# invictus717/MetaTransformer

Measured on AMD Instinct MI355X. Metric: encoder samples/sec at B=256,N=197,C=768 (Base), higher is better.
Workload: dtype bf16; 1 GPU; BASELINE config 2: Meta-Transformer-Base forward+backward+AdamW, tokens [256,197,768] bf16 per GPU, 12L/768d/12h, fp32 master weights, random init N(0,0.02); mode=train, per_gpu_batch=256, global_batch=256, parallelism=single

## Files before the change

### include/metaenc.h

```cpp
#ifndef METAENC_H
#define METAENC_H

#include <stddef.h>
#include <stdint.h>

#ifdef __cplusplus
extern "C" {
#endif

#define ME_ABI_VERSION 1

enum { ME_F32 = 0, ME_BF16 = 1,
       ME_F16 = 2 ,
       ME_BF16X3 = 3 ,
       ME_BF16X2 = 4 ,
       ME_GG8 = 5  };

enum { ME_OK = 0, ME_ERR_ARG = -1, ME_ERR_UNSUPPORTED = -2, ME_ERR_HIP = -3, ME_ERR_WORKSPACE = -4 };

int me_abi_version(void);
const char* me_last_error(void);
const char* me_build_arch(void);
int me_device_info(int dev, int* num_cus, int* lds_bytes, int* clock_mhz, char* name, int name_len);

int me_row_stats(const void* x, int x_dtype, float* out, int64_t rows, int cols, float eps, void* stream);
size_t me_row_stats_partial_bytes(int64_t rows, int cols);
int me_row_stats_combine(const float* partials, int64_t rows, int cols, float eps, float* out, void* stream);
int me_layernorm_fwd(const void* x, int x_dtype, const float* gamma, const float* beta,
                     void* y, int y_dtype, float* mean, float* rstd,
                     int64_t rows, int cols, float eps, void* stream);

size_t me_layernorm_bwd_workspace(int cols);
int me_layernorm_bwd(const void* dy, int dy_dtype, const void* x, int x_dtype,
                     const float* mean, const float* rstd, const float* gamma,
                     const void* dres, int dres_dtype, void* dx, int dx_dtype,
                     float* dgamma, float* dbeta, int accumulate_affine,
                     int64_t rows, int cols, void* workspace, void* stream);

enum { ME_GEMM_NT = 0, ME_GEMM_TN = 1 };
enum { ME_ACT_NONE = 0, ME_ACT_GELU = 1 };
enum { ME_GEMM_SAVE_GELU_GRAD = 1, ME_GEMM_AUX_IS_FACTOR = 2 };

typedef struct me_gemm_desc {
    int32_t op;
    int32_t ab_dtype;
    int64_t M, N, K;
    const void* A; int64_t lda;
    const void* B; int64_t ldb;
    void* C; int64_t ldc; int32_t c_dtype;
    int32_t act;
    float alpha, beta;
    const float* bias;
    const float* colscale;
    void* preact; int64_t ldpre; int32_t preact_dtype;
    int32_t aux_dtype;
    const void* aux; int64_t ldaux;
    const void* residual; int64_t ldres; int32_t res_dtype;
    int32_t flags;
    int64_t res_row_mod;
    int64_t out_group_rows, out_group_stride, out_row_offset;
    void* workspace; int64_t workspace_bytes;
    float* colsum_a;
    const float* row_affine;
    const float* col_shift;
    float* row_stats;
    const float* row_parts;
    int32_t row_nparts;
    float row_eps;
    int64_t a_wrap_k;
} me_gemm_desc;

size_t me_gemm_workspace_bytes(const me_gemm_desc* d);
int me_gemm_fuses_colsum(const me_gemm_desc* d);
int me_gemm_emits_row_stats(const me_gemm_desc* d);
int me_gemm_reserve_cus(int cus);
int me_gemm_takes_gg8(const me_gemm_desc* d);
int me_gemm_takes_a_wrap(const me_gemm_desc* d);
int me_gemm_takes_row_parts(const me_gemm_desc* d);
int me_gemm(const me_gemm_desc* d, void* stream);

enum { ME_PROF_LN_FWD = 16, ME_PROF_LN_BWD = 17, ME_PROF_ATTN_FWD = 18, ME_PROF_ATTN_BWD = 19, ME_PROF_ROW_STATS = 20 };
typedef struct me_gemm_profile_rec {
    int32_t op, ab_dtype;
    int64_t M, N, K;
    float ms;
    int32_t plan;
} me_gemm_profile_rec;
enum { ME_ATTN_GENERIC = 1,
       ME_ATTN_TINY = 2,
       ME_ATTN_RING16 = 3,
       ME_ATTN_RESIDENT = 4,
       ME_ATTN_STREAM16 = 5,
       ME_ATTN_MID = 6,
       ME_ATTN_CHUNK = 7,
       ME_ATTN_X3 = 8,
       ME_ATTN_QKV = 9,
       ME_ATTN_DKDV32 = 16      };
int me_gemm_profile_enable(int on);
int me_gemm_profile_read(me_gemm_profile_rec* out, int max);
// ... 292 lines not shown
```

### metatransformer_amd/_capi.py

```python
from __future__ import annotations

import ctypes
import os
from ctypes import POINTER, c_char_p, c_float, c_int, c_int32, c_int64, c_size_t, c_void_p

import torch

_HERE = os.path.dirname(os.path.abspath(__file__))
LIB_PATH = os.path.join(_HERE, "libmetaenc.so")

ME_F32, ME_BF16, ME_F16 = 0, 1, 2
ME_BF16X3 = 3
ME_BF16X2 = 4
ME_GG8 = 5
ME_GEMM_NT, ME_GEMM_TN = 0, 1
ME_ACT_NONE, ME_ACT_GELU = 0, 1
ME_GEMM_SAVE_GELU_GRAD, ME_GEMM_AUX_IS_FACTOR = 1, 2
ME_PROF_LN_FWD, ME_PROF_LN_BWD, ME_PROF_ATTN_FWD, ME_PROF_ATTN_BWD, ME_PROF_ROW_STATS = 16, 17, 18, 19, 20
ME_COMM_ID_BYTES = 128
ME_RESIZE_BILINEAR, ME_RESIZE_BICUBIC = 0, 1
ME_POOL_MEAN, ME_POOL_MAX, ME_POOL_FIRST = 0, 1, 2
ME_GROUP_DP, ME_GROUP_DP_FJ, ME_GROUP_DP_DF, ME_GROUP_DP_FJ_DF = 0, 1, 2, 3
ME_GRAPH_BWD_INDEX, ME_GRAPH_BWD_GATHER = 1, 2


class MetaEncError(RuntimeError):
    pass


class GemmDesc(ctypes.Structure):
    _fields_ = [
        ("op", c_int32), ("ab_dtype", c_int32),
        ("M", c_int64), ("N", c_int64), ("K", c_int64),
        ("A", c_void_p), ("lda", c_int64),
        ("B", c_void_p), ("ldb", c_int64),
        ("C", c_void_p), ("ldc", c_int64), ("c_dtype", c_int32),
        ("act", c_int32),
        ("alpha", c_float), ("beta", c_float),
        ("bias", c_void_p),
        ("colscale", c_void_p),
        ("preact", c_void_p), ("ldpre", c_int64), ("preact_dtype", c_int32),
        ("aux_dtype", c_int32),
        ("aux", c_void_p), ("ldaux", c_int64),
        ("residual", c_void_p), ("ldres", c_int64), ("res_dtype", c_int32),
        ("flags", c_int32),
        ("res_row_mod", c_int64),
        ("out_group_rows", c_int64), ("out_group_stride", c_int64), ("out_row_offset", c_int64),
        ("workspace", c_void_p), ("workspace_bytes", c_int64),
        ("colsum_a", c_void_p),
        ("row_affine", c_void_p), ("col_shift", c_void_p),
        ("row_stats", c_void_p),
        ("row_parts", c_void_p), ("row_nparts", c_int32), ("row_eps", c_float),
        ("a_wrap_k", c_int64),
    ]


class PatchEmbedDesc(ctypes.Structure):
    _fields_ = ([("x", c_void_p), ("x_dtype", c_int32)]
                + [(n, c_int32) for n in ("B", "Cin", "T", "H", "W", "kt", "kh", "kw", "st", "sh", "sw")]
                + [("weight", c_void_p), ("w_dtype", c_int32), ("Cout", c_int32), ("bias", c_void_p),
                   ("pos", c_void_p), ("pos_dtype", c_int32), ("ld_pos", c_int64), ("prefix_rows", c_int32),
                   ("out", c_void_p), ("out_dtype", c_int32), ("ld_out", c_int64),
                   ("workspace", c_void_p), ("workspace_bytes", c_int64)])


class GraphDesc(ctypes.Structure):
    _fields_ = ([(n, c_void_p) for n in ("node_data", "edge_data", "edge_index", "offsets", "atom", "edge", "graph_token", "null_token",
                                         "order", "Z", "perturb")]
                + [(n, c_int32) for n in ("B", "T", "C", "Fn", "Fe", "Sn", "Se", "max_n", "atom_rows", "edge_rows")])


class HsiDesc(ctypes.Structure):
    _fields_ = ([("cube", c_void_p), ("cube_dtype", c_int32), ("row_stride", c_int64), ("pix_stride", c_int64)]
                + [(n, c_int32) for n in ("H", "W", "bands")] + [("points", c_void_p)]
                + [(n, c_int32) for n in ("B", "patch", "band_patch")])


class FbankDesc(ctypes.Structure):
    _fields_ = ([("wave", c_void_p), ("ld_wave", c_int64), ("lengths", c_void_p), ("wave2", c_void_p), ("ld_wave2", c_int64),
                 ("lengths2", c_void_p), ("lam", c_void_p)]
                + [(n, c_int32) for n in ("B", "n_samples", "n_samples2", "win", "shift", "padded", "n_mel", "mel_ld", "target_length")]
                + [(n, c_void_p) for n in ("window", "twiddle", "mel_range", "mel_weight", "freq_mask", "time_mask")]
                + [("normalize", c_int32), ("norm_mean", c_float), ("norm_std", c_float), ("out", c_void_p), ("out_dtype", c_int32),
                   ("ld_out", c_int64)])


class AttnQkvDesc(ctypes.Structure):
    _fields_ = ([("q", c_void_p), ("k", c_void_p), ("v", c_void_p), ("ld_q", c_int64), ("ld_k", c_int64), ("ld_v", c_int64),
                 ("out", c_void_p), ("ld_out", c_int64), ("lse", c_void_p),
                 ("dout", c_void_p), ("ld_dout", c_int64), ("delta", c_void_p),
                 ("dq", c_void_p), ("dk", c_void_p), ("dv", c_void_p), ("ld_dq", c_int64), ("ld_dk", c_int64), ("ld_dv", c_int64),
                 ("seed", ctypes.c_uint64)]
                + [(n, c_int32) for n in ("B", "Nq", "Nk", "H", "head_dim", "dtype", "causal")]
                + [("scale", c_float), ("p_drop", c_float)])


class GemmProfileRec(ctypes.Structure):
# ... 229 lines not shown
```

### metatransformer_amd/csrc/block.hip

```cpp
#include "gemm_host.h"
#include "attention_host.h"
#include <string.h>
#include <stdlib.h>
#include <atomic>
#include <map>
#include <mutex>

namespace {

struct SideCtx {
    hipStream_t side = nullptr;
    hipEvent_t fork[4] = {nullptr, nullptr, nullptr, nullptr}, join = nullptr;
    bool failed = false;
};
std::atomic<int> g_wgrad_overlap{1};
bool wgrad_overlap_on() { return g_wgrad_overlap.load() != 0; }
constexpr size_t kMaxSideCtx = 64;
SideCtx* side_ctx(hipStream_t main) {
    static std::mutex mu;
    static std::map<std::pair<int, hipStream_t>, SideCtx> ctxs;
    hipStreamCaptureStatus st = hipStreamCaptureStatusNone;
    if (hipStreamIsCapturing(main, &st) != hipSuccess || st != hipStreamCaptureStatusNone) return nullptr;
    int dev = 0;
    if (hipStreamGetDevice(main, &dev) != hipSuccess) (void)hipGetDevice(&dev);
    std::lock_guard<std::mutex> lock(mu);
    if (ctxs.size() >= kMaxSideCtx && ctxs.find(std::make_pair(dev, main)) == ctxs.end()) return nullptr;
    SideCtx& c = ctxs[std::make_pair(dev, main)];
    if (c.failed) return nullptr;
    if (!c.side) {
        int cur = dev;
        (void)hipGetDevice(&cur);
        if (cur != dev && hipSetDevice(dev) != hipSuccess) { c.failed = true; return nullptr; }
        bool ok = hipStreamCreateWithFlags(&c.side, hipStreamNonBlocking) == hipSuccess;
        for (int i = 0; ok && i < 4; ++i) ok = hipEventCreateWithFlags(&c.fork[i], hipEventDisableTiming) == hipSuccess;
        ok = ok && hipEventCreateWithFlags(&c.join, hipEventDisableTiming) == hipSuccess;
        if (cur != dev) (void)hipSetDevice(cur);
        if (!ok) { c.failed = true; c.side = nullptr; return nullptr; }
    }
    return &c;
}

inline size_t align256(size_t v) { return (v + 255) & ~(size_t)255; }

struct Dims {
    int64_t M;
    int C, C3, Hd, hd;
    size_t esz, rsz;
};
int get_dims(const me_block_desc* d, Dims& s, const char* fn) {
    ME_CHECK_ARG(d != nullptr, "%s: null descriptor", fn);
    ME_CHECK_ARG((me_dtype_ok(d->dtype) || d->dtype == ME_BF16X3) && me_dtype_ok(d->res_dtype), "%s: bad dtype", fn);
    ME_CHECK_ARG(d->B > 0 && d->N > 0 && d->C > 0 && d->heads > 0 && d->hidden > 0 && d->C % d->heads == 0,
                 "%s: bad shape B=%d N=%d C=%d heads=%d hidden=%d", fn, d->B, d->N, d->C, d->heads, d->hidden);
    s.M = (int64_t)d->B * d->N;
    s.C = d->C; s.C3 = 3 * d->C; s.Hd = d->hidden; s.hd = d->C / d->heads;
    s.esz = d->dtype == ME_BF16X3 ? 6 : me_dtype_size(d->dtype); s.rsz = me_dtype_size(d->res_dtype);
    return ME_OK;
}

struct Saved {
    char *xn1, *qkv, *o, *x1, *xn2, *hpre, *a;
    float *mean1, *rstd1, *mean2, *rstd2, *lse;
    size_t bytes;
};
Saved carve_saved(const me_block_desc* d, const Dims& s, void* base) {
    Saved v;
    size_t off = 0;
    char* b = reinterpret_cast<char*>(base);
    auto take = [&](size_t n) { char* p = b + off; off += align256(n); return p; };
    v.xn1 = take(s.M * s.C * s.esz);
    v.qkv = take(s.M * s.C3 * s.esz);
    v.o = take(s.M * s.C * s.esz);
    v.x1 = take(s.M * s.C * s.rsz);
    v.xn2 = take(s.M * s.C * s.esz);
    v.hpre = take(s.M * s.Hd * s.esz);
    v.a = take(s.M * s.Hd * s.esz);
    v.mean1 = reinterpret_cast<float*>(take(s.M * 4));
    v.rstd1 = reinterpret_cast<float*>(take(s.M * 4));
    v.mean2 = reinterpret_cast<float*>(take(s.M * 4));
    v.rstd2 = reinterpret_cast<float*>(take(s.M * 4));
    v.lse = reinterpret_cast<float*>(take((size_t)d->B * d->heads * d->N * 4));
    v.bytes = off;
    return v;
}

void gemm_desc(me_gemm_desc& g, int op, int dt, int64_t M, int64_t N, int64_t K, const void* A, int64_t lda, const void* B,
               int64_t ldb, void* C, int64_t ldc, int cdt) {
    memset(&g, 0, sizeof(g));
    g.op = op; g.ab_dtype = dt; g.M = M; g.N = N; g.K = K;
    g.A = A; g.lda = lda; g.B = B; g.ldb = ldb; g.C = C; g.ldc = ldc; g.c_dtype = cdt;
    g.alpha = 1.0f;
}

size_t gemm_scratch(const me_block_desc* d, const Dims& s, bool backward) {
    size_t w = 0;
    me_gemm_desc g;
    auto probe = [&](int op, int64_t M, int64_t N, int64_t K, int cdt, bool cs) {
        static char dummy_mem[64] __attribute__((aligned(64)));
        gemm_desc(g, op, d->dtype, M, N, K, dummy_mem, op == ME_GEMM_NT ? K : M, dummy_mem, op == ME_GEMM_NT ? K : N, dummy_mem, N, cdt);
        if (cs) g.colsum_a = reinterpret_cast<float*>(dummy_mem);
        const size_t b = me_gemm_workspace_bytes(&g);
        if (b > w) w = b;
    };
    probe(ME_GEMM_NT, s.M, s.C3, s.C, d->dtype, false);
    probe(ME_GEMM_NT, s.M, s.C, s.C, d->res_dtype, false);
    probe(ME_GEMM_NT, s.M, s.Hd, s.C, d->dtype, false);
    probe(ME_GEMM_NT, s.M, s.C, s.Hd, d->res_dtype, false);
    if (backward) {
        probe(ME_GEMM_NT, s.M, s.C, s.C3, d->dtype, false);
        probe(ME_GEMM_NT, s.M, s.C, s.Hd, d->dtype, false);
        probe(ME_GEMM_TN, s.C3, s.C, s.M, ME_F32, true);
        probe(ME_GEMM_TN, s.C, s.C, s.M, ME_F32, true);
        probe(ME_GEMM_TN, s.Hd, s.C, s.M, ME_F32, true);
        probe(ME_GEMM_TN, s.C, s.Hd, s.M, ME_F32, true);
    }
    return align256(w);
}

size_t aux_scratch(const Dims& s) {
    size_t a = me_layernorm_bwd_workspace(s.C), b = me_colsum_workspace(s.Hd > s.C3 ? s.Hd : s.C3);
    return align256(a > b ? a : b);
}

bool wants_fold(const me_block_desc* d) {
    return d->dtype != ME_BF16X3 && d->qkv_wf && d->fc1_wf && d->qkv_s && d->qkv_c && d->fc1_s && d->fc1_c && d->res_dtype == d->dtype;
}
size_t stats_scratch(const Dims& s) { return 2 * align256(me_row_stats_partial_bytes(s.M, s.C)) + 2 * align256((size_t)s.M * 8); }
bool emits_stats(const me_block_desc* d, const Dims& s) {
    if (!wants_fold(d) || d->gamma1 || d->gamma2 || s.C % ME_STATS_GROUP) return false;
    static char dummy_mem[64] __attribute__((aligned(64)));
    me_gemm_desc g;
    for (int64_t K : {(int64_t)s.C, (int64_t)s.Hd}) {
        gemm_desc(g, ME_GEMM_NT, d->dtype, s.M, s.C, K, dummy_mem, K, dummy_mem, K, dummy_mem, s.C, d->res_dtype);
        g.bias = reinterpret_cast<const float*>(dummy_mem);
        g.residual = dummy_mem; g.ldres = s.C; g.res_dtype = d->res_dtype;
        g.workspace = dummy_mem; g.workspace_bytes = (int64_t)1 << 40;
        if (!me_gemm_emits_row_stats(&g)) return false;
    }
    return true;
}

bool takes_parts(const me_block_desc* d, const Dims& s) {
    if (!wants_fold(d) || s.C % ME_STATS_GROUP || s.C > 4 * ME_STATS_GROUP) return false;
    static char dummy_mem[64] __attribute__((aligned(64)));
    me_gemm_desc g;
    for (int64_t N : {(int64_t)s.C3, (int64_t)s.Hd}) {
        gemm_desc(g, ME_GEMM_NT, d->dtype, s.M, N, s.C, dummy_mem, s.C, dummy_mem, s.C, dummy_mem, N, d->dtype);
        g.bias = reinterpret_cast<const float*>(dummy_mem);
        g.col_shift = reinterpret_cast<const float*>(dummy_mem);
        g.row_parts = reinterpret_cast<const float*>(dummy_mem); g.row_nparts = (int32_t)(s.C / ME_STATS_GROUP); g.row_eps = d->eps;
        if (N == s.Hd) g.act = ME_ACT_GELU;
        g.workspace = dummy_mem; g.workspace_bytes = (int64_t)1 << 40;
        if (!me_gemm_takes_row_parts(&g)) return false;
    }
    return true;
}

bool x3_two_planes(const Dims& s) {
// ... 217 lines not shown
    if (d->dtype == ME_BF16X3)
        return backward ? gemm_scratch_x3(s, true) + aux_scratch(s) + bwd_scratch_x3(d, s)
                        : gemm_scratch_x3(s, false) + carve_saved_x3(d, s, nullptr).bytes;
    size_t w = gemm_scratch(d, s, backward != 0) + aux_scratch(s);
    if (!backward) return w + carve_saved(d, s, nullptr).bytes + stats_scratch(s);
    w += align256(s.M * s.C * s.esz) * 4 + align256(s.M * s.Hd * s.esz) + align256(s.M * s.C * s.rsz) +
         align256(s.M * s.C3 * s.esz) + align256((size_t)d->B * d->heads * d->N * 4);
    w += align256(me_layernorm_bwd_workspace(s.C));
    return w + gemm_scratch(d, s, true) + aux_scratch(s);
}

extern "C" int me_block_fwd(const me_block_desc* d, const void* x, void* y, void* saved, void* workspace, size_t workspace_bytes,
                            void* stream) {
    Dims s;
    int rc = get_dims(d, s, "me_block_fwd");
    if (rc) return rc;
    ME_CHECK_ARG(x && y && workspace, "me_block_fwd: null pointer");
    ME_CHECK_ARG(d->qkv_w && d->proj_w && d->fc1_w && d->fc2_w && d->ln1_g && d->ln1_b && d->ln2_g && d->ln2_b,
                 "me_block_fwd: missing parameter");
    ME_CHECK_ARG(s.M * 2 * 4 <= 2 * (int64_t)align256(s.M * 4), "me_block_fwd: stash layout");
    ME_CHECK_ARG(workspace_bytes >= me_block_workspace_bytes(d, 0), "me_block_fwd: workspace too small");
    if (d->dtype == ME_BF16X3) return block_fwd_x3(d, s, x, y, saved, workspace, stream);
    char* ws = reinterpret_cast<char*>(workspace);
    const size_t gsz = gemm_scratch(d, s, false);
    void* gws = ws;
    const bool keep = saved != nullptr;
    Saved v = carve_saved(d, s, keep ? saved : ws + gsz + aux_scratch(s));
    const int dt = d->dtype, rdt = d->res_dtype;
    me_gemm_desc g;

    const bool fold = !keep && wants_fold(d);
    const bool stats = fold && emits_stats(d, s);
    const bool parts = fold && takes_parts(d, s);
    float* partials = reinterpret_cast<float*>(ws + gsz + aux_scratch(s) + v.bytes);
    if (fold) {
        gemm_desc(g, ME_GEMM_NT, dt, s.M, s.C3, s.C, x, s.C, d->qkv_wf, s.C, v.qkv, s.C3, dt);
        g.bias = d->qkv_c; g.col_shift = d->qkv_s;
        if (d->x_parts && parts) {
            g.row_parts = d->x_parts; g.row_nparts = (int32_t)(s.C / ME_STATS_GROUP); g.row_eps = d->eps;
        } else {
            const float* st1 = d->x_stats;
            if (d->x_parts) {
                if ((rc = me_row_stats_combine(d->x_parts, s.M, s.C, d->eps, v.mean1, stream))) return rc;
                st1 = v.mean1;
            } else if (!st1) {
                if ((rc = me_row_stats(x, rdt, v.mean1, s.M, s.C, d->eps, stream))) return rc;
                st1 = v.mean1;
            }
            g.row_affine = st1;
        }
    } else {
        rc = me_layernorm_fwd(x, rdt, d->ln1_g, d->ln1_b, v.xn1, dt, keep ? v.mean1 : nullptr, keep ? v.rstd1 : nullptr, s.M, s.C, d->eps, stream);
        if (rc) return rc;
        gemm_desc(g, ME_GEMM_NT, dt, s.M, s.C3, s.C, v.xn1, s.C, d->qkv_w, s.C, v.qkv, s.C3, dt);
        g.bias = d->qkv_b;
    }
    g.workspace = gws; g.workspace_bytes = (int64_t)gsz;
    if ((rc = me_gemm(&g, stream))) return rc;
    rc = me_attention_fwd(v.qkv, s.C3, v.o, s.C, keep ? v.lse : nullptr, d->B, d->N, d->heads, s.hd, d->scale, dt, 0.f, 0, stream);
    if (rc) return rc;
    gemm_desc(g, ME_GEMM_NT, dt, s.M, s.C, s.C, v.o, s.C, d->proj_w, s.C, v.x1, s.C, rdt);
    g.bias = d->proj_b; g.colscale = d->gamma1; g.residual = x; g.ldres = s.C; g.res_dtype = rdt;
    g.workspace = gws; g.workspace_bytes = (int64_t)gsz;
    if (stats) g.row_stats = partials;
    if ((rc = me_gemm(&g, stream))) return rc;
    if (fold) {
        gemm_desc(g, ME_GEMM_NT, dt, s.M, s.Hd, s.C, v.x1, s.C, d->fc1_wf, s.C, v.a, s.Hd, dt);
        g.bias = d->fc1_c; g.col_shift = d->fc1_s;
        if (stats && parts) {
            g.row_parts = partials; g.row_nparts = (int32_t)(s.C / ME_STATS_GROUP); g.row_eps = d->eps;
        } else {
            if (stats) rc = me_row_stats_combine(partials, s.M, s.C, d->eps, v.mean2, stream);
            else rc = me_row_stats(v.x1, rdt, v.mean2, s.M, s.C, d->eps, stream);
            if (rc) return rc;
            g.row_affine = v.mean2;
        }
    } else {
        rc = me_layernorm_fwd(v.x1, rdt, d->ln2_g, d->ln2_b, v.xn2, dt, keep ? v.mean2 : nullptr, keep ? v.rstd2 : nullptr, s.M, s.C, d->eps, stream);
        if (rc) return rc;
        gemm_desc(g, ME_GEMM_NT, dt, s.M, s.Hd, s.C, v.xn2, s.C, d->fc1_w, s.C, v.a, s.Hd, dt);
        g.bias = d->fc1_b;
    }
    g.act = ME_ACT_GELU;
    if (keep) { g.preact = v.hpre; g.ldpre = s.Hd; g.preact_dtype = dt; g.flags = ME_GEMM_SAVE_GELU_GRAD; }
    g.workspace = gws; g.workspace_bytes = (int64_t)gsz;
    if ((rc = me_gemm(&g, stream))) return rc;
    gemm_desc(g, ME_GEMM_NT, dt, s.M, s.C, s.Hd, v.a, s.Hd, d->fc2_w, s.Hd, y, s.C, rdt);
    g.bias = d->fc2_b; g.colscale = d->gamma2; g.residual = v.x1; g.ldres = s.C; g.res_dtype = rdt;
    g.workspace = gws; g.workspace_bytes = (int64_t)gsz;
    float* yp = d->y_parts ? d->y_parts : partials;
    if (stats && (d->y_stats || d->y_parts)) g.row_stats = yp;
    if ((rc = me_gemm(&g, stream))) return rc;
    if (stats && d->y_stats) return me_row_stats_combine(yp, s.M, s.C, d->eps, d->y_stats, stream);
    return ME_OK;
}

extern "C" int me_block_bwd(const me_block_desc* d, const void* x, const void* dy, const void* saved, void* dx,
                            const me_block_grads* gr, void* workspace, size_t workspace_bytes, void* stream) {
    Dims s;
    int rc = get_dims(d, s, "me_block_bwd");
    if (rc) return rc;
    ME_CHECK_ARG(x && dy && saved && dx && gr && workspace, "me_block_bwd: null pointer");
    ME_CHECK_ARG(dx != dy && dx != x, "me_block_bwd: dx must not alias dy or x");
    ME_CHECK_ARG(d->qkv_wt && d->proj_wt && d->fc1_wt && d->fc2_wt && d->ln1_g && d->ln2_g, "me_block_bwd: missing parameter");
    ME_CHECK_ARG(!d->gamma1 && !d->gamma2, "me_block_bwd: layer-scale backward is composed by the host (needs the unscaled branch outputs)");
    ME_CHECK_ARG(me_dtype_ok(gr->w_dtype), "me_block_bwd: bad gradient dtype");
    ME_CHECK_ARG(workspace_bytes >= me_block_workspace_bytes(d, 1), "me_block_bwd: workspace too small");
    if (d->dtype == ME_BF16X3) return block_bwd_x3(d, s, x, dy, saved, dx, gr, workspace, stream);
    const Saved v = carve_saved(d, s, const_cast<void*>(saved));
    const int dt = d->dtype, rdt = d->res_dtype;
    char* ws = reinterpret_cast<char*>(workspace);
    size_t off = 0;
    auto take = [&](size_t n) { char* p = ws + off; off += align256(n); return p; };
    const size_t gsz = gemm_scratch(d, s, true);
    void* gws = take(gsz);
    void* aws = take(aux_scratch(s));
    char* dy_c = take(s.M * s.C * s.esz);
    char* dh = take(s.M * s.Hd * s.esz);
    char* dxn = take(s.M * s.C * s.esz);
    char* dx1 = take(s.M * s.C * s.rsz);
    char* dx1_c = take(s.M * s.C * s.esz);
    char* dout = take(s.M * s.C * s.esz);
    char* dqkv = take(s.M * s.C3 * s.esz);
    float* delta = reinterpret_cast<float*>(take((size_t)d->B * d->heads * d->N * 4));
    void* ln2_ws = take(me_layernorm_bwd_workspace(s.C));
    void* gws2 = take(gsz);
    void* aws2 = take(aux_scratch(s));
    me_ln_fold_set folds[2];
    const float beta = gr->accumulate ? 1.0f : 0.0f;
    me_gemm_desc g;
    hipStream_t mstream = reinterpret_cast<hipStream_t>(stream);
    SideCtx* sc = wgrad_overlap_on() ? side_ctx(mstream) : nullptr;
    void* wstream = sc ? reinterpret_cast<void*>(sc->side) : stream;
    void* wgws = sc ? gws2 : gws;
    void* waws = sc ? aws2 : aws;
    bool forked = false;
    auto fork = [&](int i) -> int {
        if (!sc) return ME_OK;
        if (hipEventRecord(sc->fork[i], mstream) != hipSuccess || hipStreamWaitEvent(sc->side, sc->fork[i], 0) != hipSuccess) {
            me_set_error("me_block_bwd: event fork failed");
            return ME_ERR_HIP;
        }
        forked = true;
        return ME_OK;
    };
    auto join = [&](int rc_in) -> int {
        if (!sc || !forked) return rc_in;
        if (hipEventRecord(sc->join, sc->side) != hipSuccess || hipStreamWaitEvent(mstream, sc->join, 0) != hipSuccess) {
            if (rc_in == ME_OK) { me_set_error("me_block_bwd: event join failed"); return ME_ERR_HIP; }
        }
        return rc_in;
    };

    auto nt = [&](const void* A, int64_t K, const void* Wt, void* C, int64_t N, const void* aux) -> int {
        gemm_desc(g, ME_GEMM_NT, dt, s.M, N, K, A, K, Wt, K, C, N, dt);
        if (aux) { g.aux = aux; g.ldaux = N; g.aux_dtype = dt; g.flags = ME_GEMM_AUX_IS_FACTOR; }
        g.workspace = gws; g.workspace_bytes = (int64_t)gsz;
        return me_gemm(&g, stream);
    };
    auto wgrad = [&](int fk, const void* dOut, int64_t n_out, const void* In, int64_t n_in, void* dW, float* dB) -> int {
        if (!dW && !dB) return ME_OK;
        int r = fork(fk);
        if (r) return r;
        if (dW) {
            gemm_desc(g, ME_GEMM_TN, dt, n_out, n_in, s.M, dOut, n_out, In, n_in, dW, n_in, gr->w_dtype);
            g.beta = beta; g.workspace = wgws; g.workspace_bytes = (int64_t)gsz;
            const bool fuse = dB && me_gemm_fuses_colsum(&g);
            if (fuse) g.colsum_a = dB;
            r = me_gemm(&g, wstream);
            if (r) return r;
            if (fuse) return ME_OK;
        }
        if (dB) return me_colsum(dOut, dt, n_out, s.M, n_out, dB, gr->accumulate, waws, wstream);
        return ME_OK;
    };

    const void* dyc = dy;
    if (rdt != dt) {
        if ((rc = me_cast(dy, rdt, dy_c, dt, s.M * s.C, stream))) return rc;
        dyc = dy_c;
    }
    if ((rc = wgrad(0, dyc, s.C, v.a, s.Hd, gr->fc2_w, gr->fc2_b))) return join(rc);
    if ((rc = nt(dyc, s.C, d->fc2_wt, dh, s.Hd, v.hpre))) return join(rc);
    if ((rc = wgrad(1, dh, s.Hd, v.xn2, s.C, gr->fc1_w, gr->fc1_b))) return join(rc);
    if ((rc = nt(dh, s.Hd, d->fc1_wt, dxn, s.C, nullptr))) return join(rc);
    rc = me_ln_bwd_deferred(dxn, dt, v.x1, rdt, v.mean2, v.rstd2, d->ln2_g, dy, rdt, dx1, rdt, gr->ln2_g, gr->ln2_b, gr->accumulate, s.M,
                            s.C, ln2_ws, stream, &folds[0]);
    if (rc) return join(rc);
    const void* dx1c = dx1;
    if (rdt != dt) {
        if ((rc = me_cast(dx1, rdt, dx1_c, dt, s.M * s.C, stream))) return join(rc);
        dx1c = dx1_c;
    }
    if ((rc = wgrad(2, dx1c, s.C, v.o, s.C, gr->proj_w, gr->proj_b))) return join(rc);
    if ((rc = nt(dx1c, s.C, d->proj_wt, dout, s.C, nullptr))) return join(rc);
    rc = me_attention_bwd(v.qkv, s.C3, v.o, s.C, dout, s.C, v.lse, delta, dqkv, s.C3, d->B, d->N, d->heads, s.hd, d->scale, dt, 0.f, 0, stream);
    if (rc) return join(rc);
    if ((rc = wgrad(3, dqkv, s.C3, v.xn1, s.C, gr->qkv_w, gr->qkv_b))) return join(rc);
    if ((rc = nt(dqkv, s.C3, d->qkv_wt, dxn, s.C, nullptr))) return join(rc);
    rc = me_ln_bwd_deferred(dxn, dt, x, rdt, v.mean1, v.rstd1, d->ln1_g, dx1, rdt, dx, rdt, gr->ln1_g, gr->ln1_b, gr->accumulate, s.M, s.C,
                            aws, stream, &folds[1]);
    if (rc) return join(rc);
    return join(me_ln_bwd_fold_sets(folds, 2, s.C, stream));
}

extern "C" int me_block_bwd_overlap(int enable) {
    const int prev = wgrad_overlap_on() ? 1 : 0;
    g_wgrad_overlap.store(enable ? 1 : 0);
    return prev;
}

extern "C" int me_encoder_fwd(const me_block_desc* blocks, int n_blocks, const void* x, void* y, void* pingpong, void* workspace,
                              size_t workspace_bytes, void* stream) {
    ME_CHECK_ARG(blocks && n_blocks > 0 && x && y && workspace, "me_encoder_fwd: bad args");
    ME_CHECK_ARG(n_blocks == 1 || pingpong, "me_encoder_fwd: more than one block needs the ping-pong token buffer");
    const void* in = x;
    const float* st_in = nullptr;
    const float* parts_in = nullptr;
    for (int i = 0; i < n_blocks; ++i) {
        void* out = ((n_blocks - 1 - i) % 2 == 0) ? y : pingpong;
        me_block_desc d = blocks[i];
        Dims s;
        int rc = get_dims(&d, s, "me_encoder_fwd");
        if (rc) return rc;
        d.x_stats = st_in;
        d.y_stats = nullptr;
        d.x_parts = parts_in;
        d.y_parts = nullptr;
        const me_block_desc& nx = blocks[i + 1 < n_blocks ? i + 1 : i];
        const bool chain = i + 1 < n_blocks && emits_stats(&d, s) && wants_fold(&nx) && nx.C == d.C && nx.B == d.B && nx.N == d.N &&
                           nx.eps == d.eps && nx.hidden == d.hidden && nx.heads == d.heads && nx.dtype == d.dtype &&
                           nx.res_dtype == d.res_dtype && me_block_workspace_bytes(&nx, 0) == me_block_workspace_bytes(&d, 0) &&
                           workspace_bytes >= me_block_workspace_bytes(&d, 0);
        if (chain) {
            char* tail = reinterpret_cast<char*>(workspace) + me_block_workspace_bytes(&d, 0) - 2 * align256((size_t)s.M * 8);
            Dims sn;
            if (get_dims(&nx, sn, "me_encoder_fwd") == ME_OK && takes_parts(&nx, sn))
                d.y_parts = reinterpret_cast<float*>(tail - align256(me_row_stats_partial_bytes(s.M, s.C)));
            else
// ... 11 lines not shown
```

### metatransformer_amd/csrc/common.h

```cpp
#pragma once
constexpr int ME_POL_LN_ST = 0;
constexpr int ME_POL_LN_LD = 0;
constexpr int ME_POL_ATTN_ST = 0;
constexpr int ME_POL_SLAB = 0;
#define ME_NT_LOAD(POL, ptr) ((POL) ? __builtin_nontemporal_load(ptr) : *(ptr))
#define ME_NT_STORE(POL, val, ptr) do { if (POL) __builtin_nontemporal_store((val), (ptr)); else *(ptr) = (val); } while (0)
#include <hip/hip_runtime.h>
#include <stdint.h>
#include <stdio.h>
#include "../../include/metaenc.h"

typedef __bf16 bf16_t;
typedef __attribute__((ext_vector_type(8))) __bf16 bf16x8;
typedef __attribute__((ext_vector_type(4))) __bf16 bf16x4;
typedef __attribute__((ext_vector_type(2))) __bf16 bf16x2;
typedef __attribute__((ext_vector_type(16))) float f32x16;
typedef __attribute__((ext_vector_type(4))) float f32x4;
typedef __attribute__((ext_vector_type(2))) float f32x2;
typedef __attribute__((ext_vector_type(4))) uint32_t u32x4;
constexpr float ME_GG8_LO = -0.13f, ME_GG8_STEP = 1.26f / 255.0f;
constexpr int ME_STATS_GROUP = 256;
typedef __attribute__((ext_vector_type(2))) uint32_t u32x2;

#define ME_WAVE 64

void me_set_error(const char* fmt, ...);
#define ME_CHECK_ARG(cond, ...)                 \
    do {                                        \
        if (!(cond)) {                          \
            me_set_error(__VA_ARGS__);          \
            return ME_ERR_ARG;                  \
        }                                       \
    } while (0)
#define ME_CHECK_LAUNCH(name)                                                        \
    do {                                                                             \
        hipError_t e__ = hipGetLastError();                                          \
        if (e__ != hipSuccess) {                                                     \
            me_set_error("%s: launch failed: %s", name, hipGetErrorString(e__));     \
            return ME_ERR_HIP;                                                       \
        }                                                                            \
    } while (0)

struct OncePerDevice {
    bool done[64] = {};
    bool need() {
        int d = 0;
        if (hipGetDevice(&d) != hipSuccess || d < 0 || d >= 64) return true;
        if (done[d]) return false;
        done[d] = true;
        return true;
    }
};
template <auto Kernel, typename... Args>
int launch_kernel(const char* label, dim3 grid, int threads, size_t lds, size_t lds_max, hipStream_t stream, Args... args) {
    static OncePerDevice once;
    if (once.need()) (void)hipFuncSetAttribute(reinterpret_cast<const void*>(Kernel), hipFuncAttributeMaxDynamicSharedMemorySize, (int)lds_max);
    hipLaunchKernelGGL(Kernel, grid, dim3(threads), lds, stream, args...);
    ME_CHECK_LAUNCH(label);
    return ME_OK;
}

static inline int device_cus() {
    static int n = 0;
    if (!n) {
        int dev = 0;
        (void)hipGetDevice(&dev);
        if (hipDeviceGetAttribute(&n, hipDeviceAttributeMultiprocessorCount, dev) != hipSuccess || n <= 0) n = 256;
    }
    return n;
}

struct ProfScope {
    hipEvent_t e0 = nullptr;
    hipStream_t stream;
    int op, dt;
    int64_t M, N, K;
    int plan = 0;
    ProfScope(int op, int dt, int64_t M, int64_t N, int64_t K, hipStream_t stream);
    ~ProfScope();
};

static inline size_t me_dtype_size(int dt) { return dt == ME_F32 ? 4 : dt == ME_GG8 ? 1 : 2; }
static inline bool me_dtype_ok(int dt) { return dt == ME_F32 || dt == ME_BF16; }
static inline bool me_storage_dtype_ok(int dt) { return me_dtype_ok(dt) || dt == ME_F16; }
static inline bool me_out_dtype_ok(int dt) { return me_dtype_ok(dt) || dt == ME_BF16X3; }
static inline bool me_is_planes(int dt) { return dt == ME_BF16X3 || dt == ME_BF16X2; }
static inline bool aligned4(const void* p, int dt) { return (uintptr_t)p % (4 * me_dtype_size(dt)) == 0; }
constexpr int EW_THREADS = 256;
static inline unsigned grid_blocks(int64_t work_items) {
    int64_t b = (work_items + EW_THREADS - 1) / EW_THREADS;
    const int64_t cap = 256 * 8;
    return (unsigned)(b < 1 ? 1 : (b > cap ? cap : b));
}

constexpr int LN_FOLD_SETS = 4;
struct me_ln_fold_set { const float* partial; int nrows; float* dgamma; float* dbeta; int accumulate; };
struct me_ln_fold_batch { me_ln_fold_set set[LN_FOLD_SETS]; int cols; };
int me_ln_bwd_deferred(const void* dy, int dy_dtype, const void* x, int x_dtype, const float* mean, const float* rstd, const float* gamma,
                       const void* dres, int dres_dtype, void* dx, int dx_dtype, float* dgamma, float* dbeta, int accumulate_affine,
                       int64_t rows, int cols, void* workspace, void* stream, me_ln_fold_set* defer);
int me_ln_bwd_fold_sets(const me_ln_fold_set* sets, int n, int cols, void* stream);

__device__ __forceinline__ float bf16_bits_to_f32(uint32_t lo16) { return __uint_as_float(lo16 << 16); }

__device__ __forceinline__ float wave_sum(float v) {
#pragma unroll
    for (int o = 32; o > 0; o >>= 1) v += __shfl_xor(v, o, 64);
    return v;
}
__device__ __forceinline__ float wave_max(float v) {
#pragma unroll
    for (int o = 32; o > 0; o >>= 1) v = fmaxf(v, __shfl_xor(v, o, 64));
    return v;
}

__device__ __forceinline__ f32x4 load4_as_f32(const void* base, int dt, int64_t idx) {
    if (dt == ME_BF16) {
        u32x2 raw = *reinterpret_cast<const u32x2*>(reinterpret_cast<const uint16_t*>(base) + idx);
        f32x4 r;
        r[0] = __uint_as_float(raw[0] << 16);
        r[1] = __uint_as_float(raw[0] & 0xffff0000u);
        r[2] = __uint_as_float(raw[1] << 16);
        r[3] = __uint_as_float(raw[1] & 0xffff0000u);
        return r;
    }
    return *reinterpret_cast<const f32x4*>(reinterpret_cast<const float*>(base) + idx);
}
__device__ __forceinline__ void store4_from_f32(void* base, int dt, int64_t idx, f32x4 v) {
    if (dt == ME_BF16) {
        bf16x4 o;
        o[0] = (bf16_t)v[0]; o[1] = (bf16_t)v[1]; o[2] = (bf16_t)v[2]; o[3] = (bf16_t)v[3];
        *reinterpret_cast<bf16x4*>(reinterpret_cast<uint16_t*>(base) + idx) = o;
    } else {
        *reinterpret_cast<f32x4*>(reinterpret_cast<float*>(base) + idx) = v;
    }
}
__device__ __forceinline__ void store4_split3(uint16_t* row, int64_t cols, int64_t c, f32x4 v, bool right_operand = false) {
    bf16x4 h, l;
#pragma unroll
    for (int e = 0; e < 4; ++e) {
        h[e] = (bf16_t)v[e];
        l[e] = (bf16_t)(v[e] - (float)h[e]);
    }
    *reinterpret_cast<bf16x4*>(row + c) = h;
    *reinterpret_cast<bf16x4*>(row + cols + c) = right_operand ? h : l;
    *reinterpret_cast<bf16x4*>(row + 2 * cols + c) = right_operand ? l : h;
}
__device__ __forceinline__ void store4_split2(uint16_t* row, int64_t cols, int64_t c, f32x4 v) {
    bf16x4 h, l;
#pragma unroll
    for (int e = 0; e < 4; ++e) {
        h[e] = (bf16_t)v[e];
        l[e] = (bf16_t)(v[e] - (float)h[e]);
    }
    *reinterpret_cast<bf16x4*>(row + c) = h;
    *reinterpret_cast<bf16x4*>(row + cols + c) = l;
}

__device__ __forceinline__ float load1_as_f32(const void* base, int dt, int64_t idx) {
    if (dt == ME_BF16) return bf16_bits_to_f32(reinterpret_cast<const uint16_t*>(base)[idx]);
    return reinterpret_cast<const float*>(base)[idx];
}
__device__ __forceinline__ void store1_from_f32(void* base, int dt, int64_t idx, float v) {
    if (dt == ME_BF16) reinterpret_cast<bf16_t*>(base)[idx] = (bf16_t)v;
    else reinterpret_cast<float*>(base)[idx] = v;
// ... 113 lines not shown
```

### metatransformer_amd/csrc/gemm.hip

```cpp
#include "gemm_common.h"
#include <string.h>
#include <algorithm>
#include <atomic>

namespace {

constexpr int BM = 128;
constexpr int BN = 128;
constexpr int ROWB = 128;
constexpr int TILE_BYTES = BM * ROWB;
constexpr int NT = 256;

__device__ __forceinline__ int lds_off(int row, int byteoff) {
    const int chunk = byteoff >> 4;
    return row * ROWB + (((chunk ^ ((row >> 1) & 7)) << 4) | (byteoff & 15));
}

struct Stage { u32x4 v[4]; };

template <typename T>
__device__ __forceinline__ void load_nt(Stage& s, const T* __restrict__ S, int64_t ld, int64_t nrows, int64_t K,
                                        int64_t r0, int64_t k0, int tid) {
    constexpr int E = 16 / sizeof(T);
#pragma unroll
// ... 434 lines not shown
        pl.ksteps_per_split = nk;
        if (fam == GEMM_G3) {
            const int64_t tn_ = (d->N + 255) / 256, tiles4 = tm * tn_;
            const int SL = 256;
            const int64_t R4 = tiles4 / SL, rem4 = tiles4 - R4 * SL;
            const int nkt = (int)(d->K / 64);
            const bool resident = d->c_dtype == ME_BF16 && d->alpha == 1.0f;
            if (!resident && d->N <= 1024 && d->K >= 2048 && R4 >= 1 && rem4 * 20 >= SL && rem4 * 10 <= SL * 6 && d->res_row_mod == 0 &&
                d->out_group_rows == 0) {
                const int64_t m_main = (R4 * SL) / tn_;
                const int64_t tail_tiles = (tm - m_main) * tn_;
                int s = (int)(SL / tail_tiles);
                int ktp = (nkt + s - 1) / s;
                ktp += ktp & 1;
                if (s >= 2 && m_main >= 1 && ktp >= 2) {
                    pl.tail_rows = d->M - m_main * 256;
                    pl.tail_ksteps = ktp;
                    pl.tail_split = (nkt + ktp - 1) / ktp;
                    if (pl.tail_split >= 2) pl.ws_bytes = (size_t)pl.tail_split * (size_t)pl.tail_rows * (size_t)d->N * sizeof(float);
                    else pl.tail_rows = 0;
                }
            }
            return pl;
        }
        const int64_t tn_ = (d->N + pl.bn - 1) / pl.bn, tiles = tm * tn_;
        const int64_t R = tiles / SLOTS, rem = tiles - R * SLOTS;
        if (fam == GEMM_G2W && d->N <= 1024 && R >= 1 && rem * 20 >= SLOTS && rem * 10 <= SLOTS * 6 &&
            d->res_row_mod == 0 && d->out_group_rows == 0 && d->M % pl.bm == 0) {
            const int64_t m_main = (R * SLOTS) / tn_;
            const int64_t tail_tiles = (tm - m_main) * tn_;
            int s = (int)(SLOTS / tail_tiles);
            while (s > 1 && nk / s < 8) --s;
            if (s >= 2 && m_main >= 1) {
                pl.tail_rows = (tm - m_main) * pl.bm;
                pl.tail_ksteps = (nk + s - 1) / s;
                pl.tail_split = (nk + pl.tail_ksteps - 1) / pl.tail_ksteps;
                pl.ws_bytes = (size_t)pl.tail_split * (size_t)pl.tail_rows * (size_t)d->N * sizeof(float);
            }
        }
        if (pl.tail_rows == 0 && tiles * kSmallSplitDen <= SLOTS && nk >= (small_nt ? 64 : 16) &&
            (!small_nt || tiles <= 96 || nk >= kSmallSplitLongK)) {
            int s = (int)(SLOTS / tiles);
            while (s > 1 && nk / s < 8) --s;
            if (s >= 2) {
                pl.tail_rows = d->M;
                pl.tail_ksteps = (nk + s - 1) / s;
                pl.tail_split = (nk + pl.tail_ksteps - 1) / pl.tail_ksteps;
                pl.ws_bytes = (size_t)pl.tail_split * (size_t)d->M * (size_t)d->N * sizeof(float);
            }
        }
    }
    return pl;
}

int fill_params(const me_gemm_desc* d, GemmParams& p) {
    ME_CHECK_ARG(d != nullptr, "me_gemm: null descriptor");
    ME_CHECK_ARG(d->op == ME_GEMM_NT || d->op == ME_GEMM_TN, "me_gemm: bad op %d", d->op);
    ME_CHECK_ARG(me_dtype_ok(d->ab_dtype) && (me_out_dtype_ok(d->c_dtype) || d->c_dtype == ME_BF16X2), "me_gemm: bad dtype");
    if (me_is_planes(d->c_dtype))
        ME_CHECK_ARG(d->op == ME_GEMM_NT && d->beta == 0.0f && d->ldc >= (d->c_dtype == ME_BF16X3 ? 3 : 2) * d->N && d->out_group_rows == 0 && !d->colsum_a,
                     "me_gemm: ME_BF16X3 / ME_BF16X2 output: NT, beta = 0, ldc >= 3 N / 2 N, plain rows");
    ME_CHECK_ARG(d->a_wrap_k == 0 || (d->op == ME_GEMM_NT && d->ab_dtype == ME_BF16 && d->a_wrap_k > 0 && d->a_wrap_k % 128 == 0 && d->a_wrap_k < d->K &&
                                      d->K - d->a_wrap_k <= d->a_wrap_k && d->lda >= d->a_wrap_k),
                 "me_gemm: a_wrap_k: NT, bf16, a multiple of 128 with K / 2 <= a_wrap_k < K, lda >= a_wrap_k");
    ME_CHECK_ARG(d->M > 0 && d->N > 0 && d->K > 0, "me_gemm: empty problem M=%lld N=%lld K=%lld",
                 (long long)d->M, (long long)d->N, (long long)d->K);
    ME_CHECK_ARG(d->A && d->B && d->C, "me_gemm: null operand");
    const int E = d->ab_dtype == ME_BF16 ? 8 : 4;
    ME_CHECK_ARG(d->N % 4 == 0, "me_gemm: N=%lld must be a multiple of 4", (long long)d->N);
    ME_CHECK_ARG(d->ldc % 4 == 0, "me_gemm: ldc must be a multiple of 4");
    if (d->op == ME_GEMM_NT) {
        ME_CHECK_ARG(d->K % E == 0 && d->lda % E == 0 && d->ldb % E == 0,
                     "me_gemm(NT): K, lda, ldb must be multiples of %d elements (16 bytes)", E);
    } else {
        ME_CHECK_ARG(d->M % E == 0 && d->N % E == 0 && d->lda % E == 0 && d->ldb % E == 0,
                     "me_gemm(TN): M, N, lda, ldb must be multiples of %d elements (16 bytes)", E);
    }
    ME_CHECK_ARG(((uintptr_t)d->A | (uintptr_t)d->B | (uintptr_t)d->C) % 16 == 0, "me_gemm: operands must be 16-byte aligned");
    ME_CHECK_ARG(d->act == ME_ACT_NONE || d->act == ME_ACT_GELU, "me_gemm: bad act");
    ME_CHECK_ARG((d->flags & ~(ME_GEMM_SAVE_GELU_GRAD | ME_GEMM_AUX_IS_FACTOR)) == 0, "me_gemm: unknown flags");
    ME_CHECK_ARG(!(d->flags & ME_GEMM_SAVE_GELU_GRAD) || (d->act == ME_ACT_GELU && d->preact), "me_gemm: ME_GEMM_SAVE_GELU_GRAD needs act = GELU and preact");
    ME_CHECK_ARG(!(d->flags & ME_GEMM_AUX_IS_FACTOR) || d->aux, "me_gemm: ME_GEMM_AUX_IS_FACTOR needs aux");
    if (d->preact) ME_CHECK_ARG((me_dtype_ok(d->preact_dtype) && d->ldpre % 4 == 0) ||
                                (d->preact_dtype == ME_GG8 && d->flags == ME_GEMM_SAVE_GELU_GRAD && d->ldpre % 8 == 0 && (uintptr_t)d->preact % 8 == 0), "me_gemm: bad preact");
    if (d->aux) ME_CHECK_ARG((me_dtype_ok(d->aux_dtype) && d->ldaux % 4 == 0) ||
                             (d->aux_dtype == ME_GG8 && d->flags == ME_GEMM_AUX_IS_FACTOR && d->ldaux % 8 == 0 && (uintptr_t)d->aux % 8 == 0), "me_gemm: bad aux");
    if (d->residual) ME_CHECK_ARG(me_dtype_ok(d->res_dtype) && d->ldres % 4 == 0, "me_gemm: bad residual");
    p.A = d->A; p.B = d->B; p.C = d->C;
    p.M = d->M; p.N = d->N; p.K = d->K; p.lda = d->lda; p.ldb = d->ldb; p.ldc = d->ldc;
    p.c_dtype = d->c_dtype; p.act = d->act; p.alpha = d->alpha; p.beta = d->beta;
    p.bias = d->bias; p.colscale = d->colscale;
    p.preact = d->preact; p.ldpre = d->ldpre; p.preact_dtype = d->preact_dtype;
    p.flags = d->flags;
    p.aux = d->aux; p.ldaux = d->ldaux; p.aux_dtype = d->aux_dtype;
    p.residual = d->residual; p.ldres = d->ldres; p.res_dtype = d->res_dtype;
    p.res_row_mod = d->res_row_mod; p.out_group_rows = d->out_group_rows;
    p.out_group_stride = d->out_group_stride; p.out_row_offset = d->out_row_offset;
    p.split_k = 1; p.ksteps_per_split = 0;
    p.colsum_ws = nullptr;
    ME_CHECK_ARG((d->row_affine == nullptr && d->row_parts == nullptr) == (d->col_shift == nullptr), "me_gemm: row_affine (or row_parts) and col_shift go together");
    ME_CHECK_ARG(!d->row_affine || d->op == ME_GEMM_NT, "me_gemm: row_affine (folded LayerNorm) is defined for ME_GEMM_NT");
    p.row_affine = d->row_affine; p.col_shift = d->col_shift;
    p.row_nparts = 0; p.row_eps = 0.0f;
    p.sk_wgs = 0; p.sk_upt = 0; p.sk_levels = 0; p.sk_l1 = 0;
    p.a_wrap_kt = (int)(d->a_wrap_k / 64);
    if (d->row_parts) {
        ME_CHECK_ARG(!d->row_affine && d->col_shift && d->op == ME_GEMM_NT, "me_gemm: row_parts replaces row_affine (NT, with col_shift)");
        ME_CHECK_ARG(d->row_nparts >= 1 && d->row_nparts <= 4 && (int64_t)d->row_nparts * ME_STATS_GROUP == d->K && d->row_eps >= 0.0f,
                     "me_gemm: row_parts: row_nparts = K / 256, 1 .. 4 (see me_gemm_takes_row_parts)");
        ME_CHECK_ARG((uintptr_t)d->row_parts % 8 == 0, "me_gemm: row_parts must be 8-byte aligned");
        p.row_affine = d->row_parts; p.row_nparts = d->row_nparts; p.row_eps = d->row_eps;
    }
    ME_CHECK_ARG(!d->row_stats || (d->op == ME_GEMM_NT && d->residual && (uintptr_t)d->row_stats % 8 == 0),
                 "me_gemm: row_stats goes with ME_GEMM_NT and a residual operand (8-byte aligned)");
    p.row_stats = d->row_stats;
    p.g3_full_tiles = 0; p.g3_split = 0; p.g3_ktp = 0; p.g3_slabs = nullptr; p.slab_stride = 0; p.g3_tickets = nullptr; p.g3_half = 0;
    if (d->colsum_a) ME_CHECK_ARG(d->op == ME_GEMM_TN, "me_gemm: colsum_a is defined for ME_GEMM_TN only");
    p.tiles_m = (int)((d->M + BM - 1) / BM);
    p.tiles_n = (int)((d->N + BN - 1) / BN);
    ME_CHECK_ARG((int64_t)p.tiles_m * p.tiles_n < (1ll << 31), "me_gemm: too many tiles");
    return ME_OK;
}

struct GemmRoute {
    GemmParams p;
    GemmPlan pl;
    G3Form form;
    bool colsum_a = false;
    bool a_wrap = false;
    bool gg8 = false;
    bool row_parts = false;
    bool row_stats_kernel = false, row_stats = false;
};

int route_gemm(const me_gemm_desc* d, GemmRoute& r, bool allow_sk = true) {
    GemmParams& p = r.p;
    const int rc = fill_params(d, p);
    if (rc) return rc;
    const GemmPlan& pl = r.pl = plan_gemm(d, p, allow_sk);
    if (pl.family != GEMM_G128) {
        p.tiles_m = (int)((d->M + pl.bm - 1) / pl.bm);
        p.tiles_n = (int)((d->N + pl.bn - 1) / pl.bn);
    }
    r.colsum_a = d->op == ME_GEMM_TN && ((pl.family == GEMM_G2B && pl.split_k > 1) || pl.family == GEMM_G3);
    if (pl.family != GEMM_G3 || d->op != ME_GEMM_NT) return ME_OK;
    const int cus = g3_cu_count();
    r.form = g3_form(p, cus);
    r.a_wrap = r.form.kernel == G3_ONE_TILE_WRAP;
    r.gg8 = pl.tail_rows == 0 && r.form.kernel == G3_RESIDENT && r.form.pre == G3_PRE_GG8;
    GemmParams pu = p;
    pu.a_wrap_kt = 0;
    const G3Form fu = g3_form(pu, cus);
    const bool resident = pl.tail_rows == 0 && fu.kernel == G3_RESIDENT;
    r.row_parts = resident && fu.pre == G3_PRE_ROW_PARTS && p.M * 8 * 16 < (1ll << 31);
    r.row_stats_kernel = resident && fu.repi == 2;
    r.row_stats = r.row_stats_kernel && p.res_dtype == ME_BF16 && p.N % 256 == 0 && p.M * 8 < (1ll << 31);
    return ME_OK;
}

GemmParams tail_rows_of(const GemmParams& p, int64_t m1) {
    GemmParams pt = p;
    pt.M = p.M - m1;
    pt.C = reinterpret_cast<char*>(p.C) + (size_t)m1 * p.ldc * me_dtype_size(p.c_dtype);
    if (p.preact) pt.preact = reinterpret_cast<char*>(p.preact) + (size_t)m1 * p.ldpre * me_dtype_size(p.preact_dtype);
    if (p.aux) pt.aux = reinterpret_cast<const char*>(p.aux) + (size_t)m1 * p.ldaux * me_dtype_size(p.aux_dtype);
    if (p.residual) pt.residual = reinterpret_cast<const char*>(p.residual) + (size_t)m1 * p.ldres * me_dtype_size(p.res_dtype);
    if (p.row_affine) pt.row_affine = p.row_affine + 2 * m1;
    return pt;
}

int gemm_impl(const me_gemm_desc* d, hipStream_t stream, int* plan_out, GemmTnLaunch tn_launch = nullptr, const void* tn_ctx = nullptr) {
    GemmRoute r;
    int rc = route_gemm(d, r, tn_launch == nullptr);
    if (rc) return rc;
    GemmParams& p = r.p;
    const GemmPlan& pl = r.pl;
    if (tn_launch && !(pl.family == GEMM_G3 && d->op == ME_GEMM_TN)) return ME_ERR_UNSUPPORTED;
    const bool have_ws = pl.ws_bytes && d->workspace && (size_t)d->workspace_bytes >= pl.ws_bytes;
    float* const ws = reinterpret_cast<float*>(d->workspace);
    {
        const int parts = pl.split_k > 1 ? pl.split_k : (pl.tail_rows > 0 ? pl.tail_split : 1);
        *plan_out = (pl.family & 15) | ((have_ws && parts > 1) ? 16 : 0) | (pl.sk_wgs ? 32 : 0) | ((have_ws ? parts : 1) << 8);
    }
    if (d->colsum_a)
        ME_CHECK_ARG(r.colsum_a && have_ws, "me_gemm: colsum_a needs the split-K wgrad kernel and its workspace (see me_gemm_fuses_colsum)");
    if (d->row_stats)
        ME_CHECK_ARG(d->a_wrap_k ? pl.family == GEMM_G3 && d->op == ME_GEMM_NT && pl.tail_rows == 0 : r.row_stats_kernel,
                     "me_gemm: row_stats is not available for this problem (see me_gemm_emits_row_stats)");
    if (d->a_wrap_k)
        ME_CHECK_ARG(r.a_wrap, "me_gemm: a_wrap_k is not available for this problem (see me_gemm_takes_a_wrap)");
    if (d->row_parts)
        ME_CHECK_ARG(r.row_parts, "me_gemm: row_parts is not available for this problem (see me_gemm_takes_row_parts)");
    if ((d->preact && d->preact_dtype == ME_GG8) || (d->aux && d->aux_dtype == ME_GG8))
        ME_CHECK_ARG(r.gg8, "me_gemm: ME_GG8 is not available for this problem (see me_gemm_takes_gg8)");

    if (pl.family == GEMM_G3 && d->op == ME_GEMM_TN) {
        ME_CHECK_ARG(have_ws, "me_gemm(TN, g3): workspace of me_gemm_workspace_bytes() required");
        GemmParams ps = p;
        ps.C = ws;
        ps.split_k = pl.split_k;
        ps.ksteps_per_split = pl.ksteps_per_split;
        ps.slab_stride = g3_tn_slab_stride(d->M, d->N);
        if (d->colsum_a) ps.colsum_ws = ws + (size_t)pl.split_k * (size_t)ps.slab_stride;
        if (pl.sk_wgs) {
            ps.sk_wgs = pl.sk_wgs; ps.sk_upt = pl.sk_upt; ps.sk_levels = pl.sk_levels; ps.sk_l1 = pl.sk_l1;
            rc = launch_g3_tn_sk(ps, stream);
            p.sk_wgs = pl.sk_wgs; p.sk_upt = pl.sk_upt; p.sk_levels = pl.sk_levels; p.sk_l1 = pl.sk_l1;
        } else {
            rc = tn_launch ? tn_launch(ps, stream, tn_ctx) : launch_g3_tn(ps, stream);
        }
        if (rc) return rc;
        launch_splitk_reduce(p, stream, ws, pl.split_k, ps.colsum_ws, pl.split_k * p.tiles_n, d->colsum_a, ps.slab_stride);
        ME_CHECK_LAUNCH("me_gemm(g3 tn fold)");
        return ME_OK;
    }
    if (pl.family == GEMM_G3) {
        if (!(pl.tail_rows > 0 && have_ws)) return launch_g3(p, r.form, stream);
        const int64_t m1 = d->M - pl.tail_rows;
        p.g3_full_tiles = (int)(m1 / 256) * p.tiles_n;
        p.g3_split = pl.tail_split;
        p.g3_ktp = pl.tail_ksteps;
        p.g3_slabs = ws;
        rc = launch_g3(p, g3_form(p, g3_cu_count()), stream);
        if (rc) return rc;
        GemmParams pt = tail_rows_of(p, m1);
        pt.A = nullptr;
        launch_splitk_reduce(pt, stream, ws, pl.tail_split, nullptr, 0, nullptr);
        ME_CHECK_LAUNCH("me_gemm(g3 tail fold)");
        return ME_OK;
    }
    if (pl.family == GEMM_G128) {
        if (d->ab_dtype == ME_BF16)
            return d->op == ME_GEMM_NT ? launch_g128<bf16_t, false>(p, stream) : launch_g128<bf16_t, true>(p, stream);
        return d->op == ME_GEMM_NT ? launch_g128<float, false>(p, stream) : launch_g128<float, true>(p, stream);
    }
    auto run = [&](const GemmParams& q) { return launch_g2b(q, d->op, pl.bm, pl.bn, stream); };
    p.ksteps_per_split = pl.ksteps_per_split;
    if (pl.split_k > 1 && have_ws) {
        GemmParams ps = p;
        ps.C = ws;
        ps.split_k = pl.split_k;
        if (d->colsum_a) ps.colsum_ws = ws + (size_t)pl.split_k * (size_t)d->M * (size_t)d->N;
        rc = run(ps);
        if (rc) return rc;
        launch_splitk_reduce(p, stream, ws, pl.split_k, ps.colsum_ws, pl.split_k * p.tiles_n, d->colsum_a);
        ME_CHECK_LAUNCH("me_gemm(splitk reduce)");
        return ME_OK;
    }
    p.ksteps_per_split = (int)(d->K / pl.kstep);
    if (!(pl.tail_rows > 0 && have_ws)) return run(p);
    const int64_t m1 = d->M - pl.tail_rows;
    if (m1 > 0) {
        GemmParams pm = p;
        pm.M = m1;
        pm.tiles_m = (int)(m1 / pl.bm);
        rc = run(pm);
        if (rc) return rc;
    }
    GemmParams pt = tail_rows_of(p, m1);
    pt.tiles_m = (int)((pl.tail_rows + pl.bm - 1) / pl.bm);
    pt.A = reinterpret_cast<const char*>(p.A) + (size_t)m1 * p.lda * me_dtype_size(d->ab_dtype);
    GemmParams ps = pt;
    ps.C = ws;
    ps.split_k = pl.tail_split;
    ps.ksteps_per_split = pl.tail_ksteps;
    rc = run(ps);
    if (rc) return rc;
    launch_splitk_reduce(pt, stream, ws, pl.tail_split, nullptr, 0, nullptr);
    ME_CHECK_LAUNCH("me_gemm(tail fold)");
    return ME_OK;
}

}

int gemm_fill_params(const me_gemm_desc* d, GemmParams& p) { return fill_params(d, p); }

extern "C" int me_gemm(const me_gemm_desc* d, void* stream_) {
// ... 53 lines not shown
```

### metatransformer_amd/csrc/gemm3.hip

```cpp
#include "gemm3_core.h"

namespace {
constexpr int G3_ROWOP_AHEAD = 4;
constexpr int G3_ROWOP_AHEAD_HALF = 4;
constexpr int G3_ROWOP_AHEAD_STATS = 4;

template <int EPI, bool WRAP = false>
__global__ __launch_bounds__(512) __attribute__((amdgpu_waves_per_eu(2, 2))) void gemm_g3_kernel(const GemmParams p) {
    extern __shared__ __attribute__((aligned(16))) char smem[];
    const int tid = threadIdx.x, lane = tid & 63;
    const int wave = __builtin_amdgcn_readfirstlane(tid >> 6);
    const int wr = wave >> 2;

    const int nwg = gridDim.x, bid = blockIdx.x;
    const int xcd = bid & 7, slot = bid >> 3;
    const int F = p.g3_full_tiles;
    const int nf = (F >> 3) + (xcd < (F & 7) ? 1 : 0);
    const int base_f = xcd * (F >> 3) + (xcd < (F & 7) ? xcd : (F & 7));
    int tile, part = -1;
    if (slot < nf) {
        tile = base_f + slot;
    } else {
        const int base_all = xcd * (nwg >> 3) + (xcd < (nwg & 7) ? xcd : (nwg & 7));
        const int tid_ = base_all - base_f + (slot - nf);
// ... 64 lines not shown
    (void)lane;
    lane = g3_lane_now();
    const int col = tn * G3_BN + (wave & 3) * 64 + 4 * (lane >> 4);
#pragma unroll
    for (int nt = 0; nt < 4; ++nt)
        b.v[nt] = __builtin_bit_cast(f32x4, __builtin_amdgcn_raw_buffer_load_b128(brs, (col + nt * 16) * 4, 0, 0));
    return b;
}
__device__ __forceinline__ void g3r_set_binit(G3State& s, const G3Bias& b, bool zero) {
    const f32x4 z = {0.f, 0.f, 0.f, 0.f};
#pragma unroll
    for (int j = 0; j < 4; ++j) s.binit[j] = zero ? z : b.v[j];
    asm volatile("" ::"v"(s.binit[0]), "v"(s.binit[1]), "v"(s.binit[2]), "v"(s.binit[3]));
}

__device__ __forceinline__ void g3r_rows8(f32x4& x0, f32x4& x1, f32x4& y0, f32x4& y1) {
#pragma unroll
    for (int e = 0; e < 4; ++e) {
        const unsigned a0 = __float_as_uint(x0[e]), a1 = __float_as_uint(x1[e]), b0 = __float_as_uint(y0[e]), b1 = __float_as_uint(y1[e]);
        x0[e] = __uint_as_float(__builtin_amdgcn_update_dpp(a0, b0, 0x128, 0xf, 0xc, false));
        x1[e] = __uint_as_float(__builtin_amdgcn_update_dpp(a1, b1, 0x128, 0xf, 0xc, false));
        y0[e] = __uint_as_float(__builtin_amdgcn_update_dpp(b0, a0, 0x128, 0xf, 0x3, false));
        y1[e] = __uint_as_float(__builtin_amdgcn_update_dpp(b1, a1, 0x128, 0xf, 0x3, false));
    }
}

__device__ __forceinline__ void g3r_rows8_packed(u32x4& x, u32x4& y) {
#pragma unroll
    for (int e = 0; e < 4; ++e) {
        const unsigned a = x[e], b = y[e];
        x[e] = __builtin_amdgcn_update_dpp(a, b, 0x128, 0xf, 0xc, false);
        y[e] = __builtin_amdgcn_update_dpp(b, a, 0x128, 0xf, 0x3, false);
    }
}

__device__ __forceinline__ u32x4 g3r_lanes(const u32x4& v, int addr) {
    u32x4 o;
#pragma unroll
    for (int e = 0; e < 4; ++e) o[e] = (unsigned)__builtin_amdgcn_ds_bpermute(addr, (int)v[e]);
    return o;
}

struct G3Parts { f32x4 v; };
__device__ __forceinline__ G3Parts g3r_parts_load(const GemmParams& p, int64_t m0, int rows, int wave) {
    G3Parts o;
    const int lane = g3_lane_now();
    const int t = wave * 64 + lane, rp = t >> 2, j = t & 3;
    const __amdgpu_buffer_rsrc_t pars = __builtin_amdgcn_make_buffer_rsrc(const_cast<float*>(p.row_affine) + (rows > 0 ? m0 * 2 : 0), 0,
                                                                           rows > 0 ? (int)((((int64_t)p.row_nparts - 1) * p.M + rows) * 8) : 0, 0x00020000);
    const uint32_t off = (j < p.row_nparts && 2 * rp < rows) ? (uint32_t)(((int64_t)j * p.M + 2 * rp) * 8) : 0x80000000u;
    o.v = __builtin_bit_cast(f32x4, __builtin_amdgcn_raw_buffer_load_b128(pars, (int)off, 0, 0));
    return o;
}
__device__ __forceinline__ void g3r_parts_fold(const GemmParams& p, const G3Parts& q, int wave, uint32_t lds_pairs) {
    const int lane = g3_lane_now();
    const int t = wave * 64 + lane, rp = t >> 2, j = t & 3;
    auto quad = [](float x) {
        x += __uint_as_float(__builtin_amdgcn_update_dpp(0u, __float_as_uint(x), 0xB1, 0xf, 0xf, true));
        x += __uint_as_float(__builtin_amdgcn_update_dpp(0u, __float_as_uint(x), 0x4E, 0xf, 0xf, true));
        return x;
    };
    const float w = j < p.row_nparts ? 1.0f : 0.0f;
    const float inv_np = __builtin_amdgcn_rcpf((float)p.row_nparts);
    const float inv_c = inv_np * (1.0f / 256.0f);
    u32x4 out;
#pragma unroll
    for (int r = 0; r < 2; ++r) {
        const float mean = quad(q.v[2 * r]) * inv_np;
        const float m2 = quad(q.v[2 * r + 1]);
        const float d = (q.v[2 * r] - mean) * w;
        const float dev = quad(d * d);
        const float rstd = __builtin_amdgcn_rsqf((m2 + 256.0f * dev) * inv_c + p.row_eps);
        out[2 * r] = __float_as_uint(rstd);
        out[2 * r + 1] = __float_as_uint(-rstd * mean);
    }
    asm volatile("ds_write_b128 %0, %1\n\ts_waitcnt lgkmcnt(0)" ::"v"(lds_pairs + (uint32_t)rp * 16), "v"(out) : "memory");
}

template <int EPI, int PRE, bool HALF = false>
__device__ __forceinline__ void g3_epilogue_r(const GemmParams& p, G3State& s, int64_t m0, int tn, int lane, const G3Src& nxt, int nk,
                                              const __amdgpu_buffer_rsrc_t brs, int ntn, bool next_zero, unsigned* ctr, int nx,
                                              uint32_t lds_tick, int64_t next_m0 = 0, int next_rows = 0, int par = 0) {
    constexpr bool G8 = PRE == 6, G8S = G8 && EPI == 1, G8L = G8 && EPI == 6;
    static_assert(!G8 || EPI == 1 || EPI == 6, "8-bit gelu': the fc1 forward that saves it, the fc2 dgrad that reads it");
    constexpr bool SAVE = PRE == 1 || PRE == 2 || G8S, LNF = PRE == 3 || PRE == 5, LNP = PRE == 5, STATS = PRE == 4;
    static_assert(!STATS || EPI == 2, "row statistics: the residual epilogue");
    constexpr int NMT = HALF ? 4 : 8, WROWS = HALF ? 64 : 128;
    unsigned drawn = 0;
    if (ctr && s.wave == 0) drawn = g3r_draw(ctr);
    (void)lane;
    lane = g3_lane_now();
    const int wr = s.wave >> 2, wc = s.wave & 3;
    const int r = lane & 15, g = lane >> 4;
    const int64_t n0 = (int64_t)tn * G3_BN;
    int64_t rows = p.M - m0, cols = p.N - n0;
    rows = rows < 2 * WROWS ? rows : 2 * WROWS;
    rows = rows < 1 ? 1 : rows;
    cols = cols < G3_BN ? cols : G3_BN;
    const bool item_ok = p.M > m0;
    auto tile_rsrc = [&](const void* base, int64_t ld, int esz = 2) {
        if (!item_ok) return __builtin_amdgcn_make_buffer_rsrc(const_cast<void*>(base), 0, 0, 0x00020000);
        return __builtin_amdgcn_make_buffer_rsrc(const_cast<char*>(reinterpret_cast<const char*>(base)) + (m0 * ld + n0) * esz, 0,
                                                 (int)(((rows - 1) * ld + cols) * esz), 0x00020000);
    };
    const __amdgpu_buffer_rsrc_t crs = tile_rsrc(p.C, p.ldc);
    const __amdgpu_buffer_rsrc_t prs = SAVE ? tile_rsrc(p.preact, p.ldpre, G8S ? 1 : 2) : crs;
    const __amdgpu_buffer_rsrc_t rrs = EPI == 2 ? tile_rsrc(p.residual, p.ldres) : (EPI == 3 || EPI == 6) ? tile_rsrc(p.aux, p.ldaux, G8L ? 1 : 2) : crs;
    const int rop_ld = (int)(EPI == 2 ? p.ldres : p.ldaux);
    const int colb = wc * 128 + (lane & 7) * 16;
    const bool ok = (colb >> 1) + 8 <= (int)cols;
    const int row = wr * WROWS + (lane >> 3);
    const uint32_t coff = ok ? (uint32_t)(row * (int)p.ldc * 2 + colb) : 0x80000000u;
    const uint32_t poff = ok && SAVE ? (G8S ? (uint32_t)(row * (int)p.ldpre + (colb >> 1)) : (uint32_t)(row * (int)p.ldpre * 2 + colb)) : 0x80000000u;
    const uint32_t roff = ok ? (G8L ? (uint32_t)(row * rop_ld + (colb >> 1)) : (uint32_t)(row * rop_ld * 2 + colb)) : 0x80000000u;
    const int cstep = (int)p.ldc * 16, pstep = (int)p.ldpre * (G8S ? 8 : 16), rstep = rop_ld * (G8L ? 8 : 16);
    const int to_mem = 4 * ((lane >> 3) + 8 * ((lane >> 2) & 1) + 16 * (((lane >> 1) & 1) | ((lane & 1) << 1)));
    const int to_reg = 4 * (8 * (r & 7) + 4 * (r >> 3) + 2 * (g & 1) + (g >> 1));
    auto fetch = [&](const int mt, u32x4 (&raw)[2]) {
#pragma unroll
        for (int h = 0; h < 2; ++h) {
            if (G8L) {
                const u32x2 t = __builtin_amdgcn_raw_buffer_load_b64(rrs, (int)(roff + (2 * mt + h) * rstep), 0, G3_POL_R);
                raw[h] = u32x4{t[0], t[1], 0u, 0u};
            } else {
                raw[h] = __builtin_amdgcn_raw_buffer_load_b128(rrs, (int)(roff + (2 * mt + h) * rstep), 0, G3_POL_R);
            }
        }
    };
    auto unpack8 = [](const u32x4& rw, f32x4& a, f32x4& b) {
        const f32x4 qa = {(float)(rw[0] & 0xffu), (float)((rw[0] >> 8) & 0xffu), (float)((rw[0] >> 16) & 0xffu), (float)(rw[0] >> 24)};
        const f32x4 qb = {(float)(rw[1] & 0xffu), (float)((rw[1] >> 8) & 0xffu), (float)((rw[1] >> 16) & 0xffu), (float)(rw[1] >> 24)};
        a = qa * ME_GG8_STEP + ME_GG8_LO;
        b = qb * ME_GG8_STEP + ME_GG8_LO;
    };
    auto pack8 = [](const f32x4& a, const f32x4& b) {
        unsigned w0 = 0u, w1 = 0u;
#pragma unroll
        for (int e = 0; e < 4; ++e) {
            w0 = __builtin_amdgcn_cvt_pk_u8_f32(__builtin_fmaf(a[e], 1.0f / ME_GG8_STEP, -ME_GG8_LO / ME_GG8_STEP), e, w0);
            w1 = __builtin_amdgcn_cvt_pk_u8_f32(__builtin_fmaf(b[e], 1.0f / ME_GG8_STEP, -ME_GG8_LO / ME_GG8_STEP), e, w1);
        }
        return u32x4{w0, w1, 0u, 0u};
    };
    auto lanes2 = [](const u32x4& v, int addr) {
        u32x4 o = {0u, 0u, 0u, 0u};
        o[0] = (unsigned)__builtin_amdgcn_ds_bpermute(addr, (int)v[0]);
        o[1] = (unsigned)__builtin_amdgcn_ds_bpermute(addr, (int)v[1]);
        return o;
    };
    auto unpack = [](const u32x4& rw, f32x4& a, f32x4& b) {
        a[0] = __uint_as_float(rw[0] << 16); a[1] = __uint_as_float(rw[0] & 0xffff0000u);
        a[2] = __uint_as_float(rw[1] << 16); a[3] = __uint_as_float(rw[1] & 0xffff0000u);
        b[0] = __uint_as_float(rw[2] << 16); b[1] = __uint_as_float(rw[2] & 0xffff0000u);
        b[2] = __uint_as_float(rw[3] << 16); b[3] = __uint_as_float(rw[3] & 0xffff0000u);
    };
    auto pack = [](const f32x4& a, const f32x4& b) {
        bf16x8 o;
        o[0] = (bf16_t)a[0]; o[1] = (bf16_t)a[1]; o[2] = (bf16_t)a[2]; o[3] = (bf16_t)a[3];
        o[4] = (bf16_t)b[0]; o[5] = (bf16_t)b[1]; o[6] = (bf16_t)b[2]; o[7] = (bf16_t)b[3];
        return __builtin_bit_cast(u32x4, o);
    };
    float st_a[2][3], st_b[2][3];
    __amdgpu_buffer_rsrc_t srs = crs;
    const uint32_t lds_stats = lds_tick + 64;
    if (STATS) {
        const bool part_ok = item_ok && ((int64_t)tn + 1) * 256 <= p.N;
        srs = __builtin_amdgcn_make_buffer_rsrc(p.row_stats + (part_ok ? ((int64_t)tn * p.M + m0) * 2 : 0), 0, part_ok ? (int)(rows * 8) : 0, 0x00020000);
    }
    constexpr int AHEAD = HALF ? G3_ROWOP_AHEAD_HALF : (EPI == 3 || STATS) ? G3_ROWOP_AHEAD_STATS : G3_ROWOP_AHEAD;
    u32x4 rowop[8][2];
    if (EPI == 2 || EPI == 3 || EPI == 6) {
#pragma unroll
        for (int mt = 0; mt < AHEAD; ++mt) fetch(mt, rowop[mt]);
    }
    f32x2 lnf_row[8];
    G3Bias lnf_s, lnf_c;
    G3Parts lnp;
    u32x2 lnq[8];
    if (LNF) {
        const __amdgpu_buffer_rsrc_t srs = __builtin_amdgcn_make_buffer_rsrc(const_cast<float*>(p.col_shift), 0, (int)(p.N * 4), 0x00020000);
        if (LNP) {
            const uint32_t pa = lds_tick + 64 + (uint32_t)par * 2048 + (uint32_t)(wr * WROWS + r) * 8;
#define G3R_PAIR(i) if ((i) < NMT) asm volatile("ds_read_b64 %0, %1 offset:%2" : "=v"(lnq[i]) : "v"(pa), "i"((i) * 128) : "memory");
            G3R_PAIR(0) G3R_PAIR(1) G3R_PAIR(2) G3R_PAIR(3) G3R_PAIR(4) G3R_PAIR(5) G3R_PAIR(6) G3R_PAIR(7)
#undef G3R_PAIR
            lnp = g3r_parts_load(p, next_m0, next_rows, s.wave);
        } else {
            const __amdgpu_buffer_rsrc_t rars = __builtin_amdgcn_make_buffer_rsrc(const_cast<float*>(p.row_affine) + m0 * 2, 0, item_ok ? (int)(rows * 8) : 0, 0x00020000);
#pragma unroll
            for (int mt = 0; mt < NMT; ++mt)
                lnf_row[mt] = __builtin_bit_cast(f32x2, __builtin_amdgcn_raw_buffer_load_b64(rars, (wr * WROWS + mt * 16 + r) * 8, 0, 0));
        }
        lnf_s = g3r_bias(srs, tn, s.wave, lane);
        lnf_c = g3r_bias(brs, tn, s.wave, lane);
    }
    if (HALF) g3_issue<2>(s, nxt, 1, nk);
    else g3_issue<3>(s, nxt, 1, nk);
    const G3Bias nb = g3r_bias(brs, ntn, s.wave, lane);
    __builtin_amdgcn_sched_barrier(0);
    if (LNP) {
        if (NMT == 8) asm volatile("s_waitcnt lgkmcnt(0)" : "+v"(lnq[0]), "+v"(lnq[1]), "+v"(lnq[2]), "+v"(lnq[3]), "+v"(lnq[4]), "+v"(lnq[5]), "+v"(lnq[6]), "+v"(lnq[7])::"memory");
        else asm volatile("s_waitcnt lgkmcnt(0)" : "+v"(lnq[0]), "+v"(lnq[1]), "+v"(lnq[2]), "+v"(lnq[3])::"memory");
#pragma unroll
        for (int mt = 0; mt < NMT; ++mt) lnf_row[mt] = __builtin_bit_cast(f32x2, lnq[mt]);
        __builtin_amdgcn_sched_barrier(0);
    }
#pragma unroll
    for (int mt = 0; mt < NMT; ++mt) {
        f32x4 ro[2][2];
        if (EPI == 2 || EPI == 3 || EPI == 6) {
            if (G8L) {
                unpack8(lanes2(rowop[mt][0], to_reg), ro[0][0], ro[0][1]);
                unpack8(lanes2(rowop[mt][1], to_reg), ro[1][0], ro[1][1]);
            } else {
                unpack(g3r_lanes(rowop[mt][0], to_reg), ro[0][0], ro[0][1]);
                unpack(g3r_lanes(rowop[mt][1], to_reg), ro[1][0], ro[1][1]);
            }
            if (mt + AHEAD < NMT) fetch(mt + AHEAD, rowop[mt + AHEAD]);
            __builtin_amdgcn_sched_barrier(0);
        }
        f32x4 v[2][2];
#pragma unroll
        for (int q = 0; q < 2; ++q) {
            v[q][0] = s.acc[mt][2 * q]; v[q][1] = s.acc[mt][2 * q + 1];
            if (LNF) {
                v[q][0] = v[q][0] * lnf_row[mt][0] + (lnf_s.v[2 * q] * lnf_row[mt][1] + lnf_c.v[2 * q]);
                v[q][1] = v[q][1] * lnf_row[mt][0] + (lnf_s.v[2 * q + 1] * lnf_row[mt][1] + lnf_c.v[2 * q + 1]);
            }
#pragma unroll
            for (int e = 0; e < 4; ++e) {
                const auto sw = __builtin_amdgcn_permlane16_swap(__float_as_uint(v[q][0][e]), __float_as_uint(v[q][1][e]), false, false);
                v[q][0][e] = __uint_as_float(sw[0]);
                v[q][1][e] = __uint_as_float(sw[1]);
            }
        }
        if ((EPI == 0 || EPI == 1) && !SAVE) {
            if (EPI == 1) {
                v[0][0] = gelu_bf16_4(v[0][0]); v[0][1] = gelu_bf16_4(v[0][1]);
                v[1][0] = gelu_bf16_4(v[1][0]); v[1][1] = gelu_bf16_4(v[1][1]);
            }
            u32x4 o0 = pack(v[0][0], v[0][1]), o1 = pack(v[1][0], v[1][1]);
            g3r_rows8_packed(o0, o1);
            __builtin_amdgcn_raw_buffer_store_b128(g3r_lanes(o0, to_mem), crs, (int)(coff + (2 * mt) * cstep), 0, G3_POL_C);
            __builtin_amdgcn_raw_buffer_store_b128(g3r_lanes(o1, to_mem), crs, (int)(coff + (2 * mt + 1) * cstep), 0, G3_POL_C);
            continue;
        }
        g3r_rows8(v[0][0], v[0][1], v[1][0], v[1][1]);
        float st_s[2], st_q[2], st_p[2];
#pragma unroll
        for (int h = 0; h < 2; ++h) {
            f32x4 v0 = v[h][0], v1 = v[h][1];
            if (EPI == 1) {
                if (PRE == 2 || G8S) {
                    f32x4 ph0, ga0, ph1, ga1;
                    phi_parts4(v0, ph0, ga0);
                    phi_parts4(v1, ph1, ga1);
                    const f32x4 d0 = ph0 + v0 * ga0 * 0.3989422804014327f, d1 = ph1 + v1 * ga1 * 0.3989422804014327f;
                    if (G8S) {
                        const u32x4 q8 = lanes2(pack8(d0, d1), to_mem);
                        __builtin_amdgcn_raw_buffer_store_b64(u32x2{q8[0], q8[1]}, prs, (int)(poff + (2 * mt + h) * pstep), 0, G3_POL_P);
                    } else {
                        __builtin_amdgcn_raw_buffer_store_b128(g3r_lanes(pack(d0, d1), to_mem), prs, (int)(poff + (2 * mt + h) * pstep), 0, G3_POL_P);
                    }
                    v0 *= ph0;
                    v1 *= ph1;
                } else {
                    if (SAVE) __builtin_amdgcn_raw_buffer_store_b128(g3r_lanes(pack(v0, v1), to_mem), prs, (int)(poff + (2 * mt + h) * pstep), 0, G3_POL_P);
                    v0 = gelu_bf16_4(v0);
                    v1 = gelu_bf16_4(v1);
                }
            }
            if (EPI == 6) { v0 *= ro[h][0]; v1 *= ro[h][1]; }
            if (EPI == 3) {
                v0 *= gelu_bf16_grad4(ro[h][0]);
                v1 *= gelu_bf16_grad4(ro[h][1]);
            }
            if (EPI == 2) { v0 += ro[h][0]; v1 += ro[h][1]; }
            const u32x4 pk = pack(v0, v1);
            if (STATS) {
                unpack(pk, v0, v1);
                unsigned pu = __float_as_uint(v0[0]);
                pu = __builtin_amdgcn_update_dpp(pu, pu, 0x128, 0xf, 0xc, false);
                pu = __builtin_amdgcn_permlane16_swap(pu, pu, false, false)[0];
                pu = __builtin_amdgcn_permlane32_swap(pu, pu, false, false)[0];
                const float P = __uint_as_float(pu);
                const f32x4 d0 = v0 - P, d1 = v1 - P;
                const f32x4 sd = d0 + d1, qd = d0 * d0 + d1 * d1;
                st_s[h] = (sd[0] + sd[1]) + (sd[2] + sd[3]);
                st_q[h] = (qd[0] + qd[1]) + (qd[2] + qd[3]);
                st_p[h] = P;
            }
            __builtin_amdgcn_raw_buffer_store_b128(g3r_lanes(pk, to_mem), crs, (int)(coff + (2 * mt + h) * cstep), 0, EPI == 2 ? G3_POL_C_RES : G3_POL_C);
        }
        if (STATS) {
            auto ror8 = [](float x) { return x + __uint_as_float(__builtin_amdgcn_update_dpp(0u, __float_as_uint(x), 0x128, 0xf, 0xf, true)); };
            const bool b3 = (lane >> 3) & 1, b4 = (lane >> 4) & 1, b5 = (lane >> 5) & 1;
            const float a_s0 = ror8(st_s[0]), a_s1 = ror8(st_s[1]), a_q0 = ror8(st_q[0]), a_q1 = ror8(st_q[1]);
            st_a[mt & 1][0] = b3 ? a_s1 : a_s0;
            st_a[mt & 1][1] = b3 ? a_q1 : a_q0;
            st_a[mt & 1][2] = b3 ? st_p[1] : st_p[0];
            if (mt & 1) {
                auto fold16 = [](float x, float y) {
                    const auto sw = __builtin_amdgcn_permlane16_swap(__float_as_uint(x), __float_as_uint(y), false, false);
                    return __uint_as_float(sw[0]) + __uint_as_float(sw[1]);
                };
                const int k = (mt >> 1) & 1;
                st_b[k][0] = fold16(st_a[0][0], st_a[1][0]);
                st_b[k][1] = fold16(st_a[0][1], st_a[1][1]);
                st_b[k][2] = b4 ? st_a[1][2] : st_a[0][2];
                if ((mt & 3) == 3) {
                    auto fold32 = [](float x, float y) {
                        const auto sw = __builtin_amdgcn_permlane32_swap(__float_as_uint(x), __float_as_uint(y), false, false);
                        return __uint_as_float(sw[0]) + __uint_as_float(sw[1]);
                    };
                    const float S = fold32(st_b[0][0], st_b[1][0]), Q = fold32(st_b[0][1], st_b[1][1]);
                    const float P = b5 ? st_b[1][2] : st_b[0][2];
                    const float ds = S * (1.0f / 64.0f);
                    const u32x2 out = {__float_as_uint(P + ds), __float_as_uint(Q - S * ds)};
                    const int srow = wr * WROWS + 16 * (4 * (mt >> 2) + 2 * (int)b5 + (int)b4) + 8 * (int)b3 + (lane & 7);
                    asm volatile("ds_write_b64 %0, %1" ::"v"(lds_stats + (uint32_t)(srow * 32 + wc * 8)), "v"(out) : "memory");
                }
            }
        }
    }
    if (STATS) {
        asm volatile("s_waitcnt lgkmcnt(0)" ::: "memory");
        __builtin_amdgcn_s_barrier();
        const int t = s.wave * 64 + lane, lr = t >> 1, h = t & 1;
        u32x4 raw;
        asm volatile("ds_read_b128 %0, %1\n\ts_waitcnt lgkmcnt(0)" : "=v"(raw) : "v"(lds_stats + (uint32_t)(lr * 32 + h * 16)) : "memory");
        const float ma = __uint_as_float(raw[0]), qa = __uint_as_float(raw[1]), mb = __uint_as_float(raw[2]), qb = __uint_as_float(raw[3]);
        const float d1 = mb - ma;
        const float m1 = (ma + mb) * 0.5f, q1 = (qa + qb) + d1 * d1 * 32.0f;
        auto swap1 = [](float x) { return __uint_as_float(__builtin_amdgcn_update_dpp(0u, __float_as_uint(x), 0xB1, 0xf, 0xf, true)); };
        const float mo = swap1(m1), qo = swap1(q1);
        const float d2 = mo - m1;
        const u32x2 tot = {__float_as_uint((m1 + mo) * 0.5f), __float_as_uint((q1 + qo) + d2 * d2 * 64.0f)};
        __builtin_amdgcn_raw_buffer_store_b64(tot, srs, h == 0 ? lr * 8 : (int)0x80000000u, 0, 0);
    }
    if (LNP) {
        __builtin_amdgcn_sched_barrier(0);
        g3r_parts_fold(p, lnp, s.wave, lds_tick + 64 + (uint32_t)(par ^ 1) * 2048);
        __builtin_amdgcn_sched_barrier(0);
    }
    if (HALF) {
        constexpr int PAD = (SAVE ? 16 : 8) + ((EPI == 2 || EPI == 6) ? 4 : EPI == 3 ? 8 : 0) ;
        const u32x4 z = {0u, 0u, 0u, 0u};
        const __amdgpu_buffer_rsrc_t none = __builtin_amdgcn_make_buffer_rsrc(p.C, 0, 0, 0x00020000);
#pragma unroll
        for (int i = 0; i < PAD; ++i) __builtin_amdgcn_raw_buffer_store_b128(z, none, 0, 0, 0);
    }
    __builtin_amdgcn_sched_barrier(0);
    g3r_set_binit(s, nb, next_zero);
    if (ctr && s.wave == 0) {
        asm volatile("s_waitcnt vmcnt(%0)" ::"n"(2 + 4 + 16 + (SAVE ? 16 : 0) + ((EPI == 2 || EPI == 3 || EPI == 6) ? (HALF ? 8 : 16) : 0)) : "memory");
        g3r_publish(drawn, ctr, nx, lds_tick);
    }
}

template <int EPI, int PRE> constexpr int g3r_seam() { return (PRE == 1 || PRE == 2 || (PRE == 6 && EPI == 1)) ? 32 : EPI >= 2 ? 20 : 16; }

template <int EPI, int PRE, bool HI = false>
__global__ __launch_bounds__(512) __attribute__((amdgpu_waves_per_eu(2, 2))) void gemm_g3r_kernel(const GemmParams p) {
    constexpr int SEAM = g3r_seam<EPI, PRE>();
    extern __shared__ __attribute__((aligned(16))) char smem[];
    const int tid = threadIdx.x, lane = tid & 63;
    const int wave = __builtin_amdgcn_readfirstlane(tid >> 6);
    const int wr = wave >> 2;

    const int bid = blockIdx.x, xcd = bid & 7, c = bid >> 3, G8 = gridDim.x >> 3;
    const int tiles = p.tiles_m * p.tiles_n, F = p.g3_full_tiles;
    const int nwork = F + (tiles - F) * 2;
    const int nf = (F >> 3) + (xcd < (F & 7) ? 1 : 0);
    const int nx = (nwork >> 3) + (xcd < (nwork & 7) ? 1 : 0);
    const int base_f = xcd * (F >> 3) + (xcd < (F & 7) ? xcd : (F & 7));
    const int base_all = xcd * (nwork >> 3) + (xcd < (nwork & 7) ? xcd : (nwork & 7));
    const int nkt = (int)(p.K / G3_BK);
    auto decode = [&](int slot, int& tile, int& part, int& kt0, int& kt1) {
        part = -1; kt0 = 0; kt1 = nkt;
        if (slot < nf) {
            tile = base_f + slot;
        } else {
            const int pi = base_all - base_f + (slot - nf);
            tile = F + (pi >> 1);
            part = pi & 1;
        }
    };
    auto src_of = [&](int tile, int part, int& tm, int& tn) {
        tm = __builtin_amdgcn_readfirstlane(tile / p.tiles_n);
        tn = tile - tm * p.tiles_n;
        return part >= 0 ? g3_make_src_half(p, tm, tn, part, wr) : g3_make_src(p, tm, tn);
    };
    const bool dyn = p.g3_tickets != nullptr;
    unsigned* const ctr = dyn ? p.g3_tickets + xcd * 16 : nullptr;
    const uint32_t lds_tick = (uint32_t)(uintptr_t)smem + G3_LDS;
    int slot = c;
    if (slot >= nx) return;

    G3State s;
    g3_init_lane(s, p, smem, wave, lane);
    const G3Src null = g3_null_src(p);
    const __amdgpu_buffer_rsrc_t brs = __builtin_amdgcn_make_buffer_rsrc(const_cast<float*>(p.bias), 0, p.bias ? (int)(p.N * 4) : 0, 0x00020000);
    auto prime = [&]() {
        const u32x4 z = {0u, 0u, 0u, 0u};
#pragma unroll
        for (int i = 0; i < SEAM; ++i) __builtin_amdgcn_raw_buffer_store_b128(z, null.a, 0, 0, 0);
    };

    unsigned drawn0 = 0;
    if (dyn && wave == 0) drawn0 = g3r_draw(ctr);

    int tile, part, kt0, kt1, tm, tn;
    decode(slot, tile, part, kt0, kt1);
    G3Src cur = src_of(tile, part, tm, tn);
    g3_issue<0>(s, cur, 0, kt0); g3_issue<1>(s, cur, 0, kt0); g3_issue<2>(s, cur, 0, kt0); g3_issue<3>(s, cur, 0, kt0);
    g3_issue<0>(s, cur, 1, kt0 + 1); g3_issue<1>(s, cur, 1, kt0 + 1); g3_issue<2>(s, cur, 1, kt0 + 1); g3_issue<3>(s, cur, 1, kt0 + 1);
    {
        const G3Bias b0 = g3r_bias(brs, tn, wave, lane);
        g3r_set_binit(s, b0, PRE == 3 || PRE == 5);
    }
    if (PRE == 5) {
        const int64_t m00 = (int64_t)tm * G3_BM + (part >= 0 ? part * 128 : 0);
        int64_t r0 = p.M - m00;
        r0 = r0 < (part >= 0 ? 128 : 256) ? r0 : (part >= 0 ? 128 : 256);
        const G3Parts q0 = g3r_parts_load(p, m00, r0 > 0 ? (int)r0 : 0, wave);
        g3r_parts_fold(p, q0, wave, lds_tick + 64);
    }
    asm volatile("s_waitcnt vmcnt(0)" ::: "memory");
    if (dyn && wave == 0) g3r_publish(drawn0, ctr, nx, lds_tick);
    prime();
    __builtin_amdgcn_s_barrier();
    if (wr == 1) __builtin_amdgcn_s_barrier();

    int item_par = 0;
    while (true) {
        int nslot = 0, ntile = tile, npart = -1, nkt0 = 0, nkt1 = 2, ntm = 0, ntn = 0;
        bool has_next = false;
        G3Src nxt = null;
        auto resolve_next = [&](int ns) {
            nslot = ns;
            has_next = ns < nx;
            if (has_next) {
                decode(nslot, ntile, npart, nkt0, nkt1);
// ... 86 lines not shown
    g3_init_lane_tn(s, p, smem, wave, lane);
    while (u0 < u1) {
        int tile, kt0, kt1, part, cs_row;
        int64_t ue;
        if (regular) {
            const int level = __builtin_amdgcn_readfirstlane(wgid / T);
            tile = wgid - level * T;
            kt0 = level * L1 * 2; kt1 = kt0 + L1 * 2;
            part = level;
            ue = u1;
        } else {
            tile = __builtin_amdgcn_readfirstlane((int)(u0 / Ul));
            const int64_t tu0 = (int64_t)tile * Ul;
            ue = u1 < tu0 + Ul ? u1 : tu0 + Ul;
            kt0 = (S * L1 + (int)(u0 - tu0)) * 2; kt1 = (S * L1 + (int)(ue - tu0)) * 2;
            part = S + (wgid - S * T) - sk_first(tile, E, Ul, TUl);
        }
        const int tm = __builtin_amdgcn_readfirstlane(tile / p.tiles_n), tn = tile - tm * p.tiles_n;
        cs_row = regular ? part * p.tiles_n + tn : S * p.tiles_n + (part - S) * p.tiles_n + tn;
        const int64_t m0 = (int64_t)tm * G3_BM, n0 = (int64_t)tn * G3_BN;
        g3_zero(s);
        G3Turn turn = g3_tn_colsum_begin(s, p, regular ? tn : (tn + p.tiles_n - ((kt0 >> 1) % p.tiles_n)) % p.tiles_n);
        g3_tn_walk(s, p, g3_make_src_tn(p, tm, tn), kt0, kt1, wr, turn);
        g3_tn_store_colsum(p, s, cs_row, m0, lane);
        g3_epilogue<5>(p, s, m0, n0, g3_lane_now(), reinterpret_cast<float*>(p.C) + (int64_t)part * p.slab_stride, 0);
        u0 = ue;
    }
}


unsigned* g3r_tickets(hipStream_t stream) {
    constexpr int SETS = 64, SET_WORDS = 8 * 16;
    struct Pool {
        unsigned* base = nullptr;
        bool failed = false;
        int next = 0;
        std::map<hipStream_t, int> idx;
    };
    static std::mutex mu;
    static std::map<int, Pool> pools;
    hipStreamCaptureStatus st = hipStreamCaptureStatusNone;
    if (hipStreamIsCapturing(stream, &st) != hipSuccess || st != hipStreamCaptureStatusNone) return nullptr;
    int dev = 0;
    if (hipStreamGetDevice(stream, &dev) != hipSuccess) (void)hipGetDevice(&dev);
    std::lock_guard<std::mutex> lock(mu);
    Pool& P = pools[dev];
    if (!P.base) {
        if (P.failed) return nullptr;
        unsigned* buf = nullptr;
        if (hipMalloc(&buf, (size_t)SETS * SET_WORDS * sizeof(unsigned)) != hipSuccess ||
            hipMemset(buf, 0, (size_t)SETS * SET_WORDS * sizeof(unsigned)) != hipSuccess) {
            P.failed = true;
            return nullptr;
        }
        P.base = buf;
    }
    auto it = P.idx.find(stream);
    if (it == P.idx.end()) {
        if (P.next >= SETS) return nullptr;
        unsigned* set = P.base + (size_t)P.next * SET_WORDS;
        if (hipMemsetAsync(set, 0, SET_WORDS * sizeof(unsigned), stream) != hipSuccess) return nullptr;
        it = P.idx.emplace(stream, P.next++).first;
    }
    return P.base + (size_t)it->second * SET_WORDS;
}

template <int EPI, int PRE> int launch3r(const GemmParams& q0, int G, hipStream_t stream) {
    constexpr bool HI = EPI == 0 || EPI == 2 || EPI == 1;
    constexpr int LDS_BYTES = G3_LDS + 64 + (PRE == 5 ? 4096 : PRE == 4 ? 8192 : 0);
    GemmParams q = q0;
    const int tiles = q.tiles_m * q.tiles_n, rem = tiles % G;
    q.g3_full_tiles = tiles; q.g3_split = 1; q.g3_half = 0;
    if (HI && tiles >= G && rem > 0 && 2 * rem <= G && q.K >= 4 * G3_BK) {
        q.g3_full_tiles = tiles - rem;
        q.g3_half = 1;
    }
    q.g3_tickets = q.K >= 4 * G3_BK ? g3r_tickets(stream) : nullptr;
    return launch_kernel<gemm_g3r_kernel<EPI, PRE, HI>>("me_gemm(g3 resident)", dim3((unsigned)G), 512, LDS_BYTES, LDS_BYTES, stream, q);
}

int launch3r_any(int epi, int pre, const GemmParams& q, int G, hipStream_t stream) {
    switch (epi) {
        case 0: return pre == G3_PRE_ROW_PARTS ? launch3r<0, G3_PRE_ROW_PARTS>(q, G, stream) : pre == G3_PRE_ROW_AFFINE ? launch3r<0, G3_PRE_ROW_AFFINE>(q, G, stream) : launch3r<0, G3_PRE_NONE>(q, G, stream);
        case 1: return pre == G3_PRE_GG8 ? launch3r<1, G3_PRE_GG8>(q, G, stream) : pre == G3_PRE_ROW_PARTS ? launch3r<1, G3_PRE_ROW_PARTS>(q, G, stream) :
                       pre == G3_PRE_ROW_AFFINE ? launch3r<1, G3_PRE_ROW_AFFINE>(q, G, stream) : pre == G3_PRE_SAVE_GELU_GRAD ? launch3r<1, G3_PRE_SAVE_GELU_GRAD>(q, G, stream) :
                       pre ? launch3r<1, G3_PRE_SAVE_PREACT>(q, G, stream) : launch3r<1, G3_PRE_NONE>(q, G, stream);
        case 2: return pre == G3_PRE_ROW_STATS ? launch3r<2, G3_PRE_ROW_STATS>(q, G, stream) : launch3r<2, G3_PRE_NONE>(q, G, stream);
        case 3: return launch3r<3, G3_PRE_NONE>(q, G, stream);
        default: return pre == G3_PRE_GG8 ? launch3r<6, G3_PRE_GG8>(q, G, stream) : launch3r<6, G3_PRE_NONE>(q, G, stream);
    }
}

template <int EPI, bool WRAP> int launch3t(const GemmParams& q, int nwg, hipStream_t stream) {
    return launch_kernel<gemm_g3_kernel<EPI, WRAP>>(WRAP ? "me_gemm(g3, wrapped A)" : "me_gemm(g3)", dim3((unsigned)nwg), 512, G3_LDS, G3_LDS, stream, q);
}

template <int EPI> int launch3e(const GemmParams& q, const G3Form& f, hipStream_t stream) {
    if constexpr (EPI == 0 || EPI == 4 || EPI == 8)
        if (f.kernel == G3_ONE_TILE_WRAP) return launch3t<EPI, true>(q, f.nwg, stream);
    return launch3t<EPI, false>(q, f.nwg, stream);
}

}

unsigned* me_work_counters(hipStream_t stream) { return g3r_tickets(stream); }

int launch_g3_tn(const GemmParams& p, hipStream_t stream) {
    const int nwg = p.tiles_m * p.tiles_n * p.split_k;
    return launch_kernel<gemm_g3tn_kernel>("me_gemm(g3 tn)", dim3((unsigned)nwg), 512, G3_LDS, G3_LDS, stream, p);
}

int launch_g3_tn_sk(const GemmParams& p, hipStream_t stream) {
    return launch_kernel<gemm_g3tn_sk_kernel>("me_gemm(g3 tn, balanced partition)", dim3((unsigned)p.sk_wgs), 512, G3_LDS, G3_LDS, stream, p);
}

bool g3_tn_supported(const GemmParams& p) {
    return p.M % 8 == 0 && p.N % 8 == 0 && p.lda % 8 == 0 && p.ldb % 8 == 0 && p.K * p.lda * 2 < (1ll << 31) &&
           p.K * p.ldb * 2 < (1ll << 31);
}

bool g3_supported(const GemmParams& p, int op) {
    if (op != ME_GEMM_NT) return false;
    if (p.K % (2 * G3_BK) != 0 || p.N % 8 != 0) return false;
    if (256 * p.lda * 2 >= (1ll << 31) || 256 * p.ldb * 2 >= (1ll << 31)) return false;
    return true;
}

int g3_cu_count() { return device_cus(); }

G3Form g3_form(const GemmParams& p, int cus) {
    G3Form f;
    const int e = pick_epi_ex(p);
    f.epi = (p.colscale && e != 2 && e != 8) || !((e >= 0 && e <= 3) || (e >= 6 && e <= 10)) ? 4 : e;
    const int EPI = f.epi, tiles = p.tiles_m * p.tiles_n;
    const bool split = p.g3_split > 1 && p.g3_slabs != nullptr;
    f.nwg = split ? p.g3_full_tiles + (tiles - p.g3_full_tiles) * p.g3_split : tiles;
    f.G = cus & ~7;
    if (p.a_wrap_kt) {
        f.kernel = (e == 0 || e == 4 || e == 8) ? G3_ONE_TILE_WRAP : G3_UNSUPPORTED;
        return f;
    }
    f.repi = EPI <= 3 ? EPI : -1;
    f.pre = (EPI == 1 && p.preact) ? G3_PRE_SAVE_PREACT : G3_PRE_NONE;
    const bool plain = p.beta == 0.0f && p.out_group_rows == 0 && p.res_row_mod == 0 && !p.colscale && !p.residual;
    if (EPI == 4 && p.row_affine && !p.flags && plain && !p.preact && !p.aux) {
        f.repi = p.act == ME_ACT_GELU ? 1 : 0;
        f.pre = p.row_nparts ? G3_PRE_ROW_PARTS : G3_PRE_ROW_AFFINE;
    }
    if (EPI == 4 && p.flags && !p.row_affine) {
        if (plain && p.flags == ME_GEMM_SAVE_GELU_GRAD && p.act == ME_ACT_GELU && p.preact && !p.aux) { f.repi = 1; f.pre = G3_PRE_SAVE_GELU_GRAD; }
        if (plain && p.flags == ME_GEMM_AUX_IS_FACTOR && p.act == ME_ACT_NONE && p.aux && (p.aux_dtype == ME_BF16 || p.aux_dtype == ME_GG8) && !p.preact) f.repi = 6;
    }
    if (EPI == 6) f.repi = 6;
    if (EPI == 7) { f.repi = 1; f.pre = G3_PRE_SAVE_GELU_GRAD; }
    if (f.repi == 1 && f.pre == G3_PRE_SAVE_GELU_GRAD && p.preact_dtype == ME_GG8) f.pre = G3_PRE_GG8;
    if (f.repi == 6 && p.aux_dtype == ME_GG8) f.pre = G3_PRE_GG8;
    if (EPI == 2 && p.row_stats) f.pre = G3_PRE_ROW_STATS;
    const int64_t ldmax = std::max(std::max(p.ldc, p.preact ? p.ldpre : 0), std::max(p.residual ? p.ldres : 0, p.aux ? p.ldaux : 0));
    const bool bf16_preact = !(f.pre == G3_PRE_SAVE_PREACT || f.pre == G3_PRE_SAVE_GELU_GRAD) || p.preact_dtype == ME_BF16;
    const bool gg8_rows = f.pre != G3_PRE_GG8 || !p.preact || p.ldpre % 8 == 0;
    const bool resident_only = p.row_stats || p.row_nparts || (p.preact && p.preact_dtype == ME_GG8) || (p.aux && p.aux_dtype == ME_GG8);
    if (f.repi >= 0 && !p.colscale && f.G >= 8 && f.nwg >= f.G && !split && p.alpha == 1.0f && p.c_dtype == ME_BF16 && bf16_preact && gg8_rows &&
        256 * ldmax * 2 < (1ll << 31))
        f.kernel = G3_RESIDENT;
    else
        f.kernel = resident_only ? G3_UNSUPPORTED : G3_ONE_TILE;
    return f;
}

int launch_g3(const GemmParams& p, const G3Form& f, hipStream_t stream) {
    if (f.kernel == G3_UNSUPPORTED) {
        me_set_error("me_gemm(g3): no kernel serves this descriptor");
        return ME_ERR_UNSUPPORTED;
    }
    GemmParams q = p;
    if (q.g3_split <= 1 || q.g3_slabs == nullptr) { q.g3_full_tiles = q.tiles_m * q.tiles_n; q.g3_split = 1; q.g3_ktp = 0; q.g3_slabs = nullptr; }
    if (f.kernel == G3_RESIDENT) return launch3r_any(f.repi, f.pre, q, f.G, stream);
    switch (f.epi) {
        case 0: return launch3e<0>(q, f, stream);
        case 1: return launch3e<1>(q, f, stream);
        case 2: return launch3e<2>(q, f, stream);
        case 3: return launch3e<3>(q, f, stream);
        case 6: return launch3e<6>(q, f, stream);
        case 7: return launch3e<7>(q, f, stream);
        case 8: return launch3e<8>(q, f, stream);
        case 9: return launch3e<9>(q, f, stream);
        case 10: return launch3e<10>(q, f, stream);
        default: return launch3e<4>(q, f, stream);
    }
}
```

### metatransformer_amd/csrc/gemm_common.h

```cpp
#pragma once
#include "common.h"
#include "gemm_host.h"

struct GemmParams {
    const void* A; const void* B; void* C;
    int64_t M, N, K, lda, ldb, ldc;
    int c_dtype, act;
    int flags;
    float alpha, beta;
    const float* bias; const float* colscale;
    void* preact; int64_t ldpre; int preact_dtype;
    const void* aux; int64_t ldaux; int aux_dtype;
    const void* residual; int64_t ldres; int res_dtype;
    int64_t res_row_mod, out_group_rows, out_group_stride, out_row_offset;
    int tiles_m, tiles_n;
    int split_k, ksteps_per_split;
    float* colsum_ws;
    int g3_full_tiles, g3_split, g3_ktp;
    float* g3_slabs;
    int g3_half;
    unsigned* g3_tickets;
    int64_t slab_stride;
    const float* row_affine;
    int row_nparts; float row_eps;
// ... 105 lines not shown
    if (p.row_affine) {
        const float ra = p.row_affine[2 * m], rb = p.row_affine[2 * m + 1];
        v0 = v0 * ra + *reinterpret_cast<const f32x4*>(p.col_shift + n) * rb;
        v1 = v1 * ra + *reinterpret_cast<const f32x4*>(p.col_shift + n + 4) * rb;
    }
    if (p.bias) {
        v0 += *reinterpret_cast<const f32x4*>(p.bias + n);
        v1 += *reinterpret_cast<const f32x4*>(p.bias + n + 4);
    }
    if (p.flags & ME_GEMM_SAVE_GELU_GRAD) {
        f32x4 d0, d1;
        gelu_erf_pair4(v0, v0, d0);
        gelu_erf_pair4(v1, v1, d1);
        store8_from_f32(p.preact, p.preact_dtype, m * p.ldpre + n, d0, d1);
    } else {
        if (p.preact) store8_from_f32(p.preact, p.preact_dtype, m * p.ldpre + n, v0, v1);
        if (p.act == ME_ACT_GELU) { v0 = gelu_for4(v0, p.c_dtype); v1 = gelu_for4(v1, p.c_dtype); }
    }
    if (p.aux) {
        f32x4 a0, a1;
        load8_as_f32(p.aux, p.aux_dtype, m * p.ldaux + n, a0, a1);
        if (p.flags & ME_GEMM_AUX_IS_FACTOR) { v0 *= a0; v1 *= a1; }
        else { v0 *= gelu_grad_for4(a0, p.c_dtype); v1 *= gelu_grad_for4(a1, p.c_dtype); }
    }
    if (p.colscale) {
        v0 *= *reinterpret_cast<const f32x4*>(p.colscale + n);
        v1 *= *reinterpret_cast<const f32x4*>(p.colscale + n + 4);
    }
    if (p.residual) {
        const int64_t rr = p.res_row_mod ? (m % p.res_row_mod) : m;
        f32x4 r0, r1;
        load8_as_f32(p.residual, p.res_dtype, rr * p.ldres + n, r0, r1);
        v0 += r0; v1 += r1;
    }
    const int64_t orow = p.out_group_rows
                             ? (m / p.out_group_rows) * p.out_group_stride + (m % p.out_group_rows) + p.out_row_offset
                             : m;
    if (p.c_dtype == ME_BF16X3) {
        uint16_t* row = reinterpret_cast<uint16_t*>(p.C) + orow * p.ldc;
        store4_split3(row, p.N, n, v0);
        store4_split3(row, p.N, n + 4, v1);
        return;
    }
    if (p.c_dtype == ME_BF16X2) {
        uint16_t* row = reinterpret_cast<uint16_t*>(p.C) + orow * p.ldc;
        store4_split2(row, p.N, n, v0);
        store4_split2(row, p.N, n + 4, v1);
        return;
    }
    if (p.beta != 0.0f) {
        f32x4 c0, c1;
        load8_as_f32(p.C, p.c_dtype, orow * p.ldc + n, c0, c1);
        v0 += p.beta * c0; v1 += p.beta * c1;
    }
    store8_from_f32(p.C, p.c_dtype, orow * p.ldc + n, v0, v1);
}

static inline int pick_epi(const GemmParams& p) {
    if (p.split_k > 1) return 5;
    if (me_is_planes(p.c_dtype)) return 4;
    if (p.flags || p.row_affine) return 4;
    if (p.beta != 0.0f || p.out_group_rows != 0 || p.res_row_mod != 0) return 4;
    const int nrow = (p.residual ? 1 : 0) + (p.aux ? 1 : 0);
    if (nrow > 1) return 4;
    if (p.act == ME_ACT_GELU) return (nrow == 0) ? 1 : 4;
    if (p.preact) return 4;
    if (p.residual) return p.res_dtype == ME_BF16 ? 2 : 4;
    if (p.aux) return p.aux_dtype == ME_BF16 ? 3 : 4;
    return 0;
}

static inline int pick_epi_ex(const GemmParams& p) {
    const int e = pick_epi(p);
    if (me_is_planes(p.c_dtype) && p.split_k <= 1 && !p.row_affine && !p.colscale && !p.residual && p.beta == 0.0f && p.out_group_rows == 0 &&
        p.res_row_mod == 0 && p.ldc % 8 == 0 && p.N % 8 == 0) {
        if (p.act == ME_ACT_GELU && !p.aux && (!p.preact ? p.flags == 0 : (p.flags == ME_GEMM_SAVE_GELU_GRAD && p.preact_dtype == ME_F32 && p.ldpre % 4 == 0)))
            return 9;
        if (p.act == ME_ACT_NONE && p.aux && p.aux_dtype == ME_F32 && p.flags == ME_GEMM_AUX_IS_FACTOR && !p.preact && p.ldaux % 4 == 0) return 10;
    }
    if (e == 4 && p.c_dtype == ME_F32 && p.residual && p.res_dtype == ME_F32 && !p.aux && !p.preact && p.act == ME_ACT_NONE && !p.flags &&
        !p.row_affine && p.beta == 0.0f && p.out_group_rows == 0 && p.res_row_mod == 0 && p.split_k <= 1 && p.ldres % 4 == 0)
        return 8;
    if (e != 4 || me_is_planes(p.c_dtype) || p.row_affine || p.colscale || p.residual || p.beta != 0.0f || p.out_group_rows != 0 || p.res_row_mod != 0) return e;
    if (p.flags == ME_GEMM_AUX_IS_FACTOR && p.act == ME_ACT_NONE && p.aux && (p.aux_dtype == ME_BF16 || p.aux_dtype == ME_GG8) && !p.preact) return 6;
    if (p.flags == ME_GEMM_SAVE_GELU_GRAD && p.act == ME_ACT_GELU && p.preact && !p.aux) return 7;
    return e;
}

enum GemmFamily : int {
    GEMM_G128 = 0,
    GEMM_G2B = 2,
    GEMM_G2W = 3,
    GEMM_G3 = 4,
};
int launch_g2b(const GemmParams& p, int op, int bm, int bn, hipStream_t stream);
bool g2b_supported(const GemmParams& p, int op);
bool g3_supported(const GemmParams& p, int op);

enum G3Kernel : int {
    G3_UNSUPPORTED = 0,
    G3_RESIDENT,
    G3_ONE_TILE,
    G3_ONE_TILE_WRAP,
};
enum G3Pre : int {
    G3_PRE_NONE = 0,
    G3_PRE_SAVE_PREACT = 1,
    G3_PRE_SAVE_GELU_GRAD = 2,
    G3_PRE_ROW_AFFINE = 3,
    G3_PRE_ROW_STATS = 4,
    G3_PRE_ROW_PARTS = 5,
    G3_PRE_GG8 = 6,
};
struct G3Form {
    G3Kernel kernel = G3_UNSUPPORTED;
    int epi = 4;
    int repi = -1, pre = G3_PRE_NONE;
    int G = 0;
    int nwg = 0;
};
G3Form g3_form(const GemmParams& p, int cus);
int g3_cu_count();
int launch_g3(const GemmParams& p, const G3Form& f, hipStream_t stream);
int launch_g3_tn(const GemmParams& p, hipStream_t stream);
int launch_g3_tn_sk(const GemmParams& p, hipStream_t stream);
bool g3_tn_supported(const GemmParams& p);
static inline int64_t g3_tn_slab_stride(int64_t M, int64_t N) { return M * N; }
```

### metatransformer_amd/encoder.py

```python
from __future__ import annotations

from typing import NamedTuple, Optional
import warnings

import torch
import torch.nn as nn

from . import _capi, ops
from ._capi import ME_ACT_GELU, ME_GEMM_AUX_IS_FACTOR, ME_GEMM_SAVE_GELU_GRAD, ME_GEMM_TN, MetaEncError
from .weight_cache import _WeightCache, _tensor_version


def _resolve_eps(norm_layer) -> float:
    probe = norm_layer(8)
    if not isinstance(probe, nn.LayerNorm):
        raise MetaEncError(f"norm_layer must build an nn.LayerNorm (got {type(probe).__name__})")
    return float(probe.eps)


class Mlp(nn.Module):

    def __init__(self, in_features, hidden_features=None, out_features=None, act_layer=nn.GELU, drop=0.):
        super().__init__()
        out_features = out_features or in_features
# ... 26 lines not shown
SEED_BRANCH2 = 3
SEED_ATTN_DROP = 4

_exact_notes = set()


def _note_exact_fp32(blk, cdt, rdt, reason: str) -> None:
    if cdt != torch.float32 or rdt != torch.float32 or reason in _exact_notes:
        return
    if not (blk.fp32_mode == "3xbf16" or blk.compute_dtype == "fp32_3xbf16"):
        return
    _exact_notes.add(reason)
    warnings.warn(f"metatransformer_amd: an fp32 Block runs on the exact-fp32 kernels although fp32_mode = '3xbf16': {reason} "
                  "(the three-product mode covers plain blocks -- no window, no stochastic path, no layer-scale gradient -- with dim and hidden "
                  "multiples of 256)", stacklevel=3)


BlockParams = NamedTuple("BlockParams", [(f, Optional[torch.Tensor]) for f in (
    "ln1_g", "ln1_b", "qkv_w", "qkv_b", "proj_w", "proj_b", "ln2_g", "ln2_b", "fc1_w", "fc1_b", "fc2_w", "fc2_b", "gamma1", "gamma2")])


def _grad_index(name: str) -> int:
    return 1 + BlockParams._fields.index(name)


class _BlockFn(torch.autograd.Function):

    @staticmethod
    def forward(ctx, x, ln1_g, ln1_b, qkv_w, qkv_b, proj_w, proj_b, ln2_g, ln2_b, fc1_w, fc1_b, fc2_w, fc2_b, gamma1, gamma2,
                blk, cdt, stoch, grad_mode, win, stats):
        params = BlockParams(*map(locals().get, BlockParams._fields))
        B, N, C = x.shape
        H = blk.attn.num_heads
        hd = C // H
        M = B * N
        in_dtype = x.dtype
        if in_dtype == torch.float16:
            x = ops.cast(x, torch.bfloat16)
        rdt = x.dtype
        cache: _WeightCache = blk._wcache
        need_grad = grad_mode and any(ctx.needs_input_grad)
        x2 = x.reshape(M, C)
        ctx.fast = False
        fp8 = bool(getattr(blk, "attn_fp8", False)) and win is None and cdt == torch.bfloat16 and hd == 64 and stoch is None
        if stoch is None and win is None and blk.c_side and not fp8 and not (need_grad and gamma1 is not None):
            x3 = blk.uses_3xbf16(cdt, rdt)
            if not x3:
                _note_exact_fp32(blk, cdt, rdt, "dim / hidden not multiples of 256")
            d, keep = _BlockFn._desc(blk, cache, cdt, rdt, B, N, C, H, params, False, fold=not need_grad and blk.fold_norm, x3=x3)
            want = keep[3] is not None and blk.chain_stats
            y, saved, ys = ops.block_fwd(d, x2, keep=need_grad, x_stats=stats.x_stats if want else None, want_stats=want)
            stats.y_stats = ys if in_dtype == rdt else None
            del keep
            if need_grad:
                ctx.save_for_backward(x2, saved, *params)
                ctx.blk, ctx.cdt, ctx.dims, ctx.in_dtype, ctx.fast, ctx.x3 = blk, cdt, (B, N, C, H, hd), in_dtype, True, x3
            return ops.cast(y, in_dtype).reshape(B, N, C)

        _note_exact_fp32(blk, cdt, rdt, "windowed attention" if win is not None else "stochastic path (drop-path / dropout)" if stoch is not None
                         else "layer-scale gradient" if (need_grad and gamma1 is not None) else "op-by-op composition (c_side = False)")
        xn1, mean1, rstd1 = ops.layernorm_fwd(x2, ln1_g, ln1_b, blk.eps, cdt, save_stats=need_grad)
        qkv = ops.gemm(xn1, cache.fwd("qkv", qkv_w, cdt), bias=qkv_b)
        p_attn = stoch[3] if stoch is not None else 0.0
        if win is None:
            o, lse = ops.attention_fwd(qkv, B, N, H, hd, blk.attn.scale, need_lse=need_grad, p_drop=p_attn, fp8=fp8,
                                       seed=stoch[2] + SEED_ATTN_DROP if stoch is not None else 0)
            o_att = o
        else:
            gh_, gw_, ws = win
            nwin = -(-gh_ // ws) * -(-gw_ // ws)
            qkv = ops.window_rows(qkv, B, gh_, gw_, ws, merge=False)
            o_att, lse = ops.attention_fwd(qkv, B * nwin, ws * ws, H, hd, blk.attn.scale, need_lse=need_grad, p_drop=p_attn,
                                           seed=stoch[2] + SEED_ATTN_DROP if stoch is not None else 0)
            o = ops.window_rows(o_att, B, gh_, gw_, ws, merge=True)
        ls_grad = need_grad and gamma1 is not None
        p_drop, p_path, seed = stoch[:3] if stoch is not None else (0.0, 0.0, 0)
        t1 = t2 = None
        if stoch is None and not ls_grad:
            x1 = ops.gemm(o, cache.fwd("proj", proj_w, cdt), bias=proj_b, residual=x2, out_dtype=rdt, colscale=gamma1)
        else:
            t1 = ops.gemm(o, cache.fwd("proj", proj_w, cdt), bias=proj_b, out_dtype=rdt, colscale=None if ls_grad else gamma1)
            x1 = ops.dropout_add(t1, x2, N, p_drop, p_path, seed + SEED_BRANCH1, colscale=gamma1 if ls_grad else None)
        xn2, mean2, rstd2 = ops.layernorm_fwd(x1, ln2_g, ln2_b, blk.eps, cdt, save_stats=need_grad)
        hpre = torch.empty((M, fc1_w.shape[0]), dtype=cdt, device=x.device) if need_grad else None
        a = ops.gemm(xn2, cache.fwd("fc1", fc1_w, cdt), bias=fc1_b, act=ME_ACT_GELU, preact=hpre,
                     flags=ME_GEMM_SAVE_GELU_GRAD if need_grad else 0)
        if stoch is None and not ls_grad:
            y = ops.gemm(a, cache.fwd("fc2", fc2_w, cdt), bias=fc2_b, residual=x1, out_dtype=rdt, colscale=gamma2)
        else:
            if p_drop > 0:
                a = ops.dropout_add(a, None, N, p_drop, 0.0, seed + SEED_MLP_HIDDEN)
            t2 = ops.gemm(a, cache.fwd("fc2", fc2_w, cdt), bias=fc2_b, out_dtype=rdt, colscale=None if ls_grad else gamma2)
            y = ops.dropout_add(t2, x1, N, p_drop, p_path, seed + SEED_BRANCH2, colscale=gamma2 if ls_grad else None)
        if not ls_grad:
            t1 = t2 = None

        if need_grad:
            ctx.save_for_backward(x2, mean1, rstd1, xn1, qkv, lse, o, x1, mean2, rstd2, xn2, hpre, a,
                                  ln1_g, qkv_w, proj_w, ln2_g, fc1_w, fc2_w, gamma1, gamma2, t1, t2, o_att if win is not None else None)
            ctx.blk, ctx.cdt, ctx.dims, ctx.stoch, ctx.win = blk, cdt, (B, N, C, H, hd), stoch, win
            ctx.has_bias = (qkv_b is not None, proj_b is not None, fc1_b is not None, fc2_b is not None)
            ctx.in_dtype = in_dtype
        return ops.cast(y, in_dtype).reshape(B, N, C)

    @staticmethod
    def _desc(blk, cache, cdt, rdt, B, N, C, H, p: BlockParams, transposed, fold=False, x3=False):
        w, wt = cache.operands({"qkv": p.qkv_w, "proj": p.proj_w, "fc1": p.fc1_w, "fc2": p.fc2_w}, cdt, x3, transposed)
        vec = {k: None if t is None else ops._f32(t).contiguous() for k, t in p._asdict().items() if not k.endswith("_w")}
        d = ops.block_desc(B, N, C, H, p.fc1_w.shape[0], blk.eps, blk.attn.scale, cdt, rdt, w, wt, vec, x3=x3)
        folded = None
        big = ((B * N + 255) // 256) * ((3 * C + 255) // 256) >= 256
        if fold and (big or fold == "always") and cdt == torch.bfloat16 and rdt == torch.bfloat16:
            folded = (cache.folded("qkv", p.qkv_w, p.ln1_g, p.ln1_b, p.qkv_b, cdt), cache.folded("fc1", p.fc1_w, p.ln2_g, p.ln2_b, p.fc1_b, cdt))
            (d.qkv_wf, d.qkv_s, d.qkv_c), (d.fc1_wf, d.fc1_s, d.fc1_c) = [tuple(ops.ptr(t) for t in trip) for trip in folded]
        return d, (w, wt, vec, folded)

    @staticmethod
    def _backward_c(ctx, dy):
        x2, saved, *params = ctx.saved_tensors
        blk, cdt = ctx.blk, ctx.cdt
        B, N, C, H, hd = ctx.dims
        rdt = x2.dtype
        ng = ctx.needs_input_grad
        dy2 = dy.contiguous().reshape(B * N, C)
        if dy2.dtype != rdt:
            dy2 = ops.cast(dy2, rdt)
        d, keep = _BlockFn._desc(blk, blk._wcache, cdt, rdt, B, N, C, H, BlockParams(*params), True, x3=ctx.x3)
        slots = [(n, p, _grad_index(n)) for n, p in blk._params()._asdict().items()
                 if p is not None and not n.startswith("gamma") and ng[_grad_index(n)]]
        flat = getattr(blk.attn.qkv.weight, "_me_flat", None)
        direct = None
        if flat is not None and slots and all(p.dtype == torch.float32 and getattr(p, "_me_flat", None) is flat for _, p, _ in slots):
            direct = [flat.direct_grad(p) for _, p, _ in slots]
            if any(t is None for t in direct):
                direct = None
        g = _capi.BlockGrads()
        wdt = blk.attn.qkv.weight.dtype
        wdt = wdt if wdt != torch.float16 else torch.float32
        g.w_dtype = _capi.dtype_code(wdt)
        g.accumulate = 1 if direct is not None else 0
        outs = {}
        for j, (n, p, i) in enumerate(slots):
            outs[i] = direct[j] if direct is not None else torch.empty(p.shape, dtype=wdt if n.endswith("_w") else torch.float32, device=p.device)
            setattr(g, n, ops.ptr(outs[i]))
        dx = ops.block_bwd(d, x2, dy2, saved, g)
        del keep
        res = [None] * len(ng)
        res[0] = ops.cast(dx, ctx.in_dtype).reshape(B, N, C) if ng[0] else None
        for n, p, i in slots:
            if direct is not None:
                flat.grad_written(p)
            else:
                t = outs[i]
                res[i] = t if t.dtype == p.dtype else (ops.cast(t, p.dtype) if t.dim() == 2 else t.to(p.dtype))
        return tuple(res)

    @staticmethod
    def backward(ctx, dy):
        if ctx.fast:
            return _BlockFn._backward_c(ctx, dy)
        (x2, mean1, rstd1, xn1, qkv, lse, o, x1, mean2, rstd2, xn2, hpre, a,
         n1w, qkvw, projw, n2w, fc1w, fc2w, g1, g2, t1, t2, o_att) = ctx.saved_tensors
        blk, cdt = ctx.blk, ctx.cdt
        B, N, C, H, hd = ctx.dims
        M = B * N
        cache: _WeightCache = blk._wcache
        rdt = x2.dtype
        ng = ctx.needs_input_grad
        need = lambda name: ng[_grad_index(name)]
        dy2 = dy.contiguous().reshape(M, C)
        if dy2.dtype != rdt:
            dy2 = ops.cast(dy2, rdt)

        def wgrad(dout, inp, lin, need_w, need_b):
            w = lin.weight
            if not need_w:
                return None, (ops.colsum(dout).to(w.dtype) if need_b else None)
            flat = getattr(w, "_me_flat", None)
            tgt = flat.direct_grad(w) if (flat is not None and w.dtype == torch.float32) else None
            tgt_b = None
            if tgt is not None and need_b and getattr(lin.bias, "_me_flat", None) is flat and lin.bias.dtype == torch.float32:
                tgt_b = flat.direct_grad(lin.bias)
            fuse_b = need_b and (tgt is None or tgt_b is not None)
            odt = w.dtype if w.dtype != torch.float16 else torch.float32
            res = ops.gemm(dout, inp, op=ME_GEMM_TN, out=tgt, out_dtype=odt, beta=1.0 if tgt is not None else 0.0,
                           want_colsum_a=fuse_b, colsum_out=tgt_b)
            dw, db = res if fuse_b else (res, ops.colsum(dout) if need_b else None)
            if tgt is not None:
                flat.grad_written(w)
                dw = None
            if tgt_b is not None:
                flat.grad_written(lin.bias)
                db = None
            if dw is not None and dw.dtype != w.dtype:
                dw = ops.cast(dw, w.dtype)
            return dw, (db.to(w.dtype) if db is not None else None)

        def ln_bwd(dyn, xin, mean, rstd, norm, dres, need_aff):
            flat = getattr(norm.weight, "_me_flat", None)
            acc = None
            if need_aff and flat is not None and getattr(norm.bias, "_me_flat", None) is flat and norm.weight.dtype == torch.float32:
                gw, gb = flat.direct_grad(norm.weight), flat.direct_grad(norm.bias)
                if gw is not None and gb is not None:
                    acc = (gw, gb)
            dxo, dg, db = ops.layernorm_bwd(dyn, xin, mean, rstd, norm.weight, dres, rdt, need_aff, affine_accum=acc)
            if acc is not None:
                flat.grad_written(norm.weight)
                flat.grad_written(norm.bias)
            return dxo, dg, db

        stoch = ctx.stoch
        p_drop, p_path, seed = stoch[:3] if stoch is not None else (0.0, 0.0, 0)
        p_attn = stoch[3] if stoch is not None else 0.0

        def branch_grad(dout, t, g, sd):
            dm = dout if stoch is None else ops.dropout_add(dout, None, N, p_drop, p_path, sd)
            if g is None:
                return ops.cast(dm, cdt), None
            dg = ops.colsum_mul(dm, t)
            return ops.dropout_add(dm, None, N, 0.0, 0.0, 0, out_dtype=cdt, colscale=g), dg

        dy_c, d_g2 = branch_grad(dy2, t2, g2, seed + SEED_BRANCH2)
        dh = ops.gemm(dy_c, cache.transposed("fc2", fc2w, cdt), aux=hpre, flags=ME_GEMM_AUX_IS_FACTOR)
        if stoch is not None and p_drop > 0:
            dh = ops.dropout_add(dh, None, N, p_drop, 0.0, seed + SEED_MLP_HIDDEN)
        d_fc2w, d_fc2b = wgrad(dy_c, a, blk.mlp.fc2, need("fc2_w"), need("fc2_b") and ctx.has_bias[3])
        dxn2 = ops.gemm(dh, cache.transposed("fc1", fc1w, cdt))
        d_fc1w, d_fc1b = wgrad(dh, xn2, blk.mlp.fc1, need("fc1_w"), need("fc1_b") and ctx.has_bias[2])
        dx1, d_n2w, d_n2b = ln_bwd(dxn2, x1, mean2, rstd2, blk.norm2, dy2, need("ln2_g") or need("ln2_b"))

        dx1_c, d_g1 = branch_grad(dx1, t1, g1, seed + SEED_BRANCH1)
        do = ops.gemm(dx1_c, cache.transposed("proj", projw, cdt))
        d_projw, d_projb = wgrad(dx1_c, o, blk.attn.proj, need("proj_w"), need("proj_b") and ctx.has_bias[1])
        if ctx.win is None:
            dqkv = ops.attention_bwd(qkv, o, do, lse, B, N, H, hd, blk.attn.scale, p_drop=p_attn, seed=seed + SEED_ATTN_DROP)
        else:
            gh_, gw_, ws = ctx.win
            nwin = -(-gh_ // ws) * -(-gw_ // ws)
            do_w = ops.window_rows(do, B, gh_, gw_, ws, merge=False)
            dqkv_w = ops.attention_bwd(qkv, o_att, do_w, lse, B * nwin, ws * ws, H, hd, blk.attn.scale, p_drop=p_attn,
                                       seed=seed + SEED_ATTN_DROP)
            dqkv = ops.window_rows(dqkv_w, B, gh_, gw_, ws, merge=True)
        dxn1 = ops.gemm(dqkv, cache.transposed("qkv", qkvw, cdt))
        d_qkvw, d_qkvb = wgrad(dqkv, xn1, blk.attn.qkv, need("qkv_w"), need("qkv_b") and ctx.has_bias[0])
        dx, d_n1w, d_n1b = ln_bwd(dxn1, x2, mean1, rstd1, blk.norm1, dx1, need("ln1_g") or need("ln1_b"))

        def vec(name, g, like):
            return g.to(like.dtype) if (g is not None and need(name)) else None

        grads = BlockParams(ln1_g=vec("ln1_g", d_n1w, n1w), ln1_b=vec("ln1_b", d_n1b, n1w), qkv_w=d_qkvw, qkv_b=d_qkvb,
                            proj_w=d_projw, proj_b=d_projb, ln2_g=vec("ln2_g", d_n2w, n2w), ln2_b=vec("ln2_b", d_n2b, n2w),
                            fc1_w=d_fc1w, fc1_b=d_fc1b, fc2_w=d_fc2w, fc2_b=d_fc2b,
                            gamma1=vec("gamma1", d_g1, g1), gamma2=vec("gamma2", d_g2, g2))
        res = [None] * len(ng)
        res[0] = ops.cast(dx, ctx.in_dtype).reshape(B, N, C) if ng[0] else None
        for name, g in grads._asdict().items():
            res[_grad_index(name)] = g
        return tuple(res)


class _StatsHandoff:
    x_stats = y_stats = None


class Block(nn.Module):

    def __init__(self, dim, num_heads, mlp_ratio=4., qkv_bias=False, qk_scale=None, drop=0., attn_drop=0.,
                 drop_path=0., act_layer=nn.GELU, norm_layer=nn.LayerNorm, layer_scale=False, windowed=False,
                 window_size=14):
        super().__init__()
        self.windowed, self.window_size = bool(windowed), int(window_size)
        self.eps = _resolve_eps(norm_layer)
        self.norm1 = nn.LayerNorm(dim, eps=self.eps)
        self.attn = Attention(dim, num_heads=num_heads, qkv_bias=qkv_bias, qk_scale=qk_scale,
                              attn_drop=attn_drop, proj_drop=drop)
        self.drop_path_prob = float(drop_path)
        self.drop_path = nn.Identity()
        self.norm2 = nn.LayerNorm(dim, eps=self.eps)
        self.mlp = Mlp(in_features=dim, hidden_features=int(dim * mlp_ratio), act_layer=act_layer, drop=drop)
        self.layer_scale = bool(layer_scale)
        if layer_scale:
            self.gamma1 = nn.Parameter(torch.ones(dim))
            self.gamma2 = nn.Parameter(torch.ones(dim))
        self.compute_dtype: Optional[torch.dtype] = None
        self.c_side = True
        self.attn_fp8 = False
        self.fold_norm = True
        self.fp32_mode = Block.default_fp32_mode
        self._wcache = _WeightCache()
        self.chain_stats = True

    default_fp32_mode = "3xbf16"

    def uses_3xbf16(self, cdt, rdt) -> bool:
        want = self.fp32_mode == "3xbf16" or self.compute_dtype == "fp32_3xbf16"
        if self.fp32_mode not in ("exact", "3xbf16"):
            raise MetaEncError(f"Block.fp32_mode must be 'exact' or '3xbf16' (got {self.fp32_mode!r})")
        C, hidden = self.attn.qkv.weight.shape[1], self.mlp.fc1.weight.shape[0]
        return bool(want and cdt == torch.float32 and rdt == torch.float32 and C % 256 == 0 and hidden % 256 == 0)

    def _params(self) -> BlockParams:
        a, m = self.attn, self.mlp
        return BlockParams(ln1_g=self.norm1.weight, ln1_b=self.norm1.bias, qkv_w=a.qkv.weight, qkv_b=a.qkv.bias, proj_w=a.proj.weight,
                           proj_b=a.proj.bias, ln2_g=self.norm2.weight, ln2_b=self.norm2.bias, fc1_w=m.fc1.weight, fc1_b=m.fc1.bias,
                           fc2_w=m.fc2.weight, fc2_b=m.fc2.bias, gamma1=self.gamma1 if self.layer_scale else None,
                           gamma2=self.gamma2 if self.layer_scale else None)
# ... 197 lines not shown
```

### metatransformer_amd/ops.py

```python
from __future__ import annotations

import ctypes
from typing import Optional, Tuple

import torch

from . import _capi
from ._capi import GemmDesc, MetaEncError, check, dtype_code, ptr, stream_ptr

WEIGHT_EPOCH = 0

def gemm_profile(on: bool) -> None:
    check(_capi.load().me_gemm_profile_enable(1 if on else 0), "me_gemm_profile_enable")


def gemm_profile_read(max_records: int = 1 << 16, with_plan: bool = False):
    lib = _capi.load()
    buf = (_capi.GemmProfileRec * max_records)()
    n = lib.me_gemm_profile_read(buf, max_records)
    if with_plan:
        return [(r.op, r.ab_dtype, r.M, r.N, r.K, r.ms, r.plan) for r in buf[:min(n, max_records)]]
    return [(r.op, r.ab_dtype, r.M, r.N, r.K, r.ms) for r in buf[:min(n, max_records)]]


def _req(t: torch.Tensor, name: str) -> torch.Tensor:
    if not isinstance(t, torch.Tensor) or not t.is_cuda:
        raise MetaEncError(f"{name}: expected a CUDA/ROCm tensor (libmetaenc has no CPU path)")
    if not t.is_contiguous():
        raise MetaEncError(f"{name}: tensor must be contiguous")
    return t


def _f32(t: Optional[torch.Tensor]) -> Optional[torch.Tensor]:
    if t is None:
        return None
    return t if t.dtype == torch.float32 else t.float()



def layernorm_fwd(x: torch.Tensor, gamma: torch.Tensor, beta: torch.Tensor, eps: float,
                  out_dtype: torch.dtype, save_stats: bool = True):
    lib = _capi.load()
    _req(x, "x")
    C = x.shape[-1]
    rows = x.numel() // C
    y = torch.empty(x.shape, dtype=out_dtype, device=x.device)
    mean = torch.empty(rows, dtype=torch.float32, device=x.device) if save_stats else None
    rstd = torch.empty(rows, dtype=torch.float32, device=x.device) if save_stats else None
    g, b = _f32(gamma).contiguous(), _f32(beta).contiguous()
    check(lib.me_layernorm_fwd(ptr(x), dtype_code(x.dtype), ptr(g), ptr(b), ptr(y), dtype_code(out_dtype),
                               ptr(mean), ptr(rstd), rows, C, float(eps), stream_ptr()), "me_layernorm_fwd")
    return y, mean, rstd


def layernorm_bwd(dy: torch.Tensor, x: torch.Tensor, mean: torch.Tensor, rstd: torch.Tensor, gamma: torch.Tensor,
                  dres: Optional[torch.Tensor], dx_dtype: torch.dtype, need_affine: bool,
                  affine_accum: Optional[Tuple[torch.Tensor, torch.Tensor]] = None):
    lib = _capi.load()
    _req(dy, "dy"); _req(x, "x")
    C = x.shape[-1]
    rows = x.numel() // C
    dx = torch.empty(x.shape, dtype=dx_dtype, device=x.device)
    g = _f32(gamma).contiguous()
    accumulate = 0
    if need_affine and affine_accum is not None:
        dgamma, dbeta = affine_accum
        accumulate = 1
    else:
        dgamma = torch.empty(C, dtype=torch.float32, device=x.device) if need_affine else None
        dbeta = torch.empty(C, dtype=torch.float32, device=x.device) if need_affine else None
    ws = None
    if need_affine:
        ws = torch.empty(lib.me_layernorm_bwd_workspace(C), dtype=torch.uint8, device=x.device)
    check(lib.me_layernorm_bwd(ptr(dy), dtype_code(dy.dtype), ptr(x), dtype_code(x.dtype), ptr(mean), ptr(rstd), ptr(g),
                               ptr(dres), dtype_code(dres.dtype) if dres is not None else 0,
                               ptr(dx), dtype_code(dx_dtype), ptr(dgamma), ptr(dbeta), accumulate, rows, C, ptr(ws),
                               stream_ptr()), "me_layernorm_bwd")
    if accumulate:
        return dx, None, None
    return dx, dgamma, dbeta



def gemm(a: torch.Tensor, b: torch.Tensor, *, op: int = _capi.ME_GEMM_NT, out: Optional[torch.Tensor] = None,
         out_dtype: Optional[torch.dtype] = None, bias: Optional[torch.Tensor] = None, act: int = _capi.ME_ACT_NONE,
         residual: Optional[torch.Tensor] = None, res_row_mod: int = 0, preact: Optional[torch.Tensor] = None,
         aux: Optional[torch.Tensor] = None, colscale: Optional[torch.Tensor] = None, alpha: float = 1.0,
         beta: float = 0.0, out_rows: Optional[int] = None, out_group: Tuple[int, int, int] = (0, 0, 0),
         want_colsum_a: bool = False, colsum_out: Optional[torch.Tensor] = None, flags: int = 0,
         row_affine: Optional[torch.Tensor] = None, col_shift: Optional[torch.Tensor] = None, want_row_stats: bool = False,
         row_parts: Optional[torch.Tensor] = None, row_eps: float = 0.0):
    lib = _capi.load()
    _req(a, "a"); _req(b, "b")
    if a.dtype != b.dtype:
        raise MetaEncError(f"gemm: operand dtypes differ ({a.dtype} vs {b.dtype})")
    a2 = a.reshape(-1, a.shape[-1])
    b2 = b.reshape(-1, b.shape[-1])
    if op == _capi.ME_GEMM_NT:
        M, K = a2.shape
        N, Kb = b2.shape
    else:
        K, M = a2.shape
        Kb, N = b2.shape
    if K != Kb:
        raise MetaEncError(f"gemm: reduction dims differ ({K} vs {Kb})")
    if out is None:
        out = torch.empty((out_rows if out_rows is not None else M, N), dtype=out_dtype or a.dtype, device=a.device)
    _req(out, "out")
    d = GemmDesc()
    d.op, d.ab_dtype = op, dtype_code(a.dtype)
    d.M, d.N, d.K = M, N, K
    d.A, d.lda = ptr(a2), a2.stride(0)
    d.B, d.ldb = ptr(b2), b2.stride(0)
    d.C, d.ldc, d.c_dtype = ptr(out), out.stride(-2), dtype_code(out.dtype)
    d.act, d.alpha, d.beta = act, alpha, beta
    d.flags = flags
    keep = []
    if row_affine is not None:
        if row_affine.dtype != torch.float32 or row_affine.shape != (M, 2) or col_shift is None or col_shift.numel() != N:
            raise MetaEncError("gemm: row_affine must be [M, 2] float32 (ops.row_stats) and col_shift [N]")
        col_shift = _f32(col_shift).contiguous(); keep.append(col_shift)
        d.row_affine, d.col_shift = ptr(_req(row_affine, "row_affine")), ptr(col_shift)
    if row_parts is not None:
        if row_affine is not None or col_shift is None or col_shift.numel() != N or row_parts.dtype != torch.float32 or \
                K % 256 or tuple(row_parts.shape) != (K // 256, M, 2):
            raise MetaEncError("gemm: row_parts must be [K / 256, M, 2] float32 partials (gemm(..., want_row_stats=True)), with col_shift [N], without row_affine")
        col_shift = _f32(col_shift).contiguous(); keep.append(col_shift)
        d.row_parts, d.row_nparts, d.row_eps, d.col_shift = ptr(_req(row_parts, "row_parts")), K // 256, float(row_eps), ptr(col_shift)
    if bias is not None:
        bias = _f32(bias).contiguous(); keep.append(bias)
        d.bias = ptr(bias)
    if colscale is not None:
        colscale = _f32(colscale).contiguous(); keep.append(colscale)
        d.colscale = ptr(colscale)
    if preact is not None:
        _req(preact, "preact")
        d.preact, d.ldpre, d.preact_dtype = ptr(preact), preact.stride(-2), _capi.ME_GG8 if preact.dtype == torch.uint8 else dtype_code(preact.dtype)
    if aux is not None:
        _req(aux, "aux")
        d.aux, d.ldaux, d.aux_dtype = ptr(aux), aux.stride(-2), _capi.ME_GG8 if aux.dtype == torch.uint8 else dtype_code(aux.dtype)
    if residual is not None:
        _req(residual, "residual")
        d.residual, d.ldres, d.res_dtype = ptr(residual), residual.stride(-2), dtype_code(residual.dtype)
        d.res_row_mod = res_row_mod
    d.out_group_rows, d.out_group_stride, d.out_row_offset = out_group
    cs = None
    if want_colsum_a:
        if op != _capi.ME_GEMM_TN:
            raise MetaEncError("gemm: want_colsum_a is defined for ME_GEMM_TN")
        if lib.me_gemm_fuses_colsum(ctypes.byref(d)):
            cs = colsum_out if colsum_out is not None else torch.empty(M, dtype=torch.float32, device=a.device)
            keep.append(cs)
            d.colsum_a = ptr(cs)

    ws_bytes = lib.me_gemm_workspace_bytes(ctypes.byref(d))
    if ws_bytes:
        ws = torch.empty(ws_bytes, dtype=torch.uint8, device=a.device); keep.append(ws)
        d.workspace, d.workspace_bytes = ptr(ws), ws_bytes
    partials = None
    if want_row_stats and lib.me_gemm_emits_row_stats(ctypes.byref(d)):
        partials = torch.empty((N // 256, M, 2), dtype=torch.float32, device=a.device)
        d.row_stats = ptr(partials)
    check(lib.me_gemm(ctypes.byref(d), stream_ptr()), "me_gemm")
    if want_row_stats:
        return out, partials
    if want_colsum_a:
        if cs is None:
            cs = colsum(a2, out=colsum_out, accumulate=beta != 0.0)
        return out, cs
    return out


GG8_LO, GG8_STEP = -0.13, 1.26 / 255.0


def gemm_takes_gg8(M: int, N: int, K: int) -> bool:
    lib = _capi.load()
    dev = torch.device("cuda", torch.cuda.current_device())
    dummy = torch.empty(64, dtype=torch.uint8, device=dev)
    for save in (True, False):
        d = GemmDesc()
        d.op, d.ab_dtype, d.c_dtype = _capi.ME_GEMM_NT, _capi.ME_BF16, _capi.ME_BF16
        d.M, d.N, d.K, d.lda, d.ldb, d.ldc = M, N, K, K, K, N
        d.A = d.B = d.C = ptr(dummy)
        d.alpha = 1.0
        if save:
            d.act, d.flags, d.preact, d.ldpre, d.preact_dtype = _capi.ME_ACT_GELU, _capi.ME_GEMM_SAVE_GELU_GRAD, ptr(dummy), N, _capi.ME_GG8
        else:
            d.flags, d.aux, d.ldaux, d.aux_dtype = _capi.ME_GEMM_AUX_IS_FACTOR, ptr(dummy), N, _capi.ME_GG8
        d.workspace, d.workspace_bytes = ptr(dummy), 1 << 40
        if not lib.me_gemm_takes_gg8(ctypes.byref(d)):
            return False
    return True


def colsum(x: torch.Tensor, out: Optional[torch.Tensor] = None, accumulate: bool = False) -> torch.Tensor:
    lib = _capi.load()
    _req(x, "x")
    x2 = x.reshape(-1, x.shape[-1])
    rows, cols = x2.shape
    if out is None:
        out, accumulate = torch.empty(cols, dtype=torch.float32, device=x.device), False
    ws = torch.empty(lib.me_colsum_workspace(cols), dtype=torch.uint8, device=x.device)
    check(lib.me_colsum(ptr(x2), dtype_code(x.dtype), x2.stride(0), rows, cols, ptr(out), 1 if accumulate else 0, ptr(ws),
                        stream_ptr()), "me_colsum")
    return out



def block_desc(B, N, C, heads, hidden, eps, scale, cdt, rdt, w, wt, vec, x3: bool = False) -> "_capi.BlockDesc":
    d = _capi.BlockDesc()
    d.dtype, d.res_dtype = (_capi.ME_BF16X3 if x3 else dtype_code(cdt)), dtype_code(rdt)
    d.B, d.N, d.C, d.heads, d.hidden, d.eps, d.scale = B, N, C, heads, hidden, eps, scale
    for k in ("qkv", "proj", "fc1", "fc2"):
        setattr(d, k + "_w", ptr(w[k]))
        setattr(d, k + "_wt", ptr(wt[k]) if wt is not None else None)
    for k, t in vec.items():
        setattr(d, k, ptr(t))
    return d


def block_fwd(d, x2: torch.Tensor, keep: bool, x_stats: Optional[torch.Tensor] = None, want_stats: bool = False):
    lib = _capi.load()
    y = torch.empty_like(x2)
    saved = torch.empty(lib.me_block_saved_bytes(ctypes.byref(d)), dtype=torch.uint8, device=x2.device) if keep else None
    wsb = lib.me_block_workspace_bytes(ctypes.byref(d), 0)
    ws = torch.empty(wsb, dtype=torch.uint8, device=x2.device)
    y_stats = None
    if not keep:
        if x_stats is not None:
            M, C = x2.shape
            if x_stats.dtype != torch.float32 or not x_stats.is_contiguous() or x_stats.device != x2.device or \
                    tuple(x_stats.shape) not in ((M, 2), (C // 256, M, 2)):
                raise MetaEncError("block_fwd: x_stats must be a contiguous float32 tensor on the tokens' device, [M, 2] pairs "
                                   "(row_stats) or the [C / 256, M, 2] partials a previous block_fwd(want_stats=True) returned")
            if x_stats.dim() == 3:
                d.x_parts = ptr(x_stats)
            else:
                d.x_stats = ptr(x_stats)
        if want_stats and lib.me_block_emits_stats(ctypes.byref(d)):
            y_stats = torch.empty((x2.shape[1] // 256, x2.shape[0], 2), dtype=torch.float32, device=x2.device)
            d.y_parts = ptr(y_stats)
    check(lib.me_block_fwd(ctypes.byref(d), ptr(x2), ptr(y), ptr(saved), ptr(ws), wsb, stream_ptr()), "me_block_fwd")
    return y, saved, y_stats


def encoder_fwd(descs, x2: torch.Tensor) -> torch.Tensor:
    lib = _capi.load()
    n = len(descs)
    arr = (_capi.BlockDesc * n)(*descs)
    y = torch.empty_like(x2)
    pp = torch.empty_like(x2) if n > 1 else None
    wsb = max(lib.me_block_workspace_bytes(ctypes.byref(d), 0) for d in descs)
    ws = torch.empty(wsb, dtype=torch.uint8, device=x2.device)
    check(lib.me_encoder_fwd(arr, n, ptr(x2), ptr(y), ptr(pp), ptr(ws), wsb, stream_ptr()), "me_encoder_fwd")
    return y


def attention_fwd_x3(qkv: torch.Tensor, B: int, N: int, H: int, hd: int, scale: float, need_lse: bool = False, planes: bool = False,
                     want_out: bool = True):
    lib = _capi.load()
    _req(qkv, "qkv")
    if qkv.dtype != torch.float32:
        raise MetaEncError("attention_fwd_x3: float32 qkv required")
    C = H * hd
    out = torch.empty((B * N, C), dtype=torch.float32, device=qkv.device) if want_out else None
    lse = torch.empty((B, H, N), dtype=torch.float32, device=qkv.device) if need_lse else None
    o3 = torch.empty((B * N, 3 * C), dtype=torch.bfloat16, device=qkv.device) if planes else None
    check(lib.me_attention_fwd_x3(ptr(qkv), qkv.stride(-2), ptr(out), C, ptr(o3), ptr(lse), B, N, H, hd, float(scale), stream_ptr()),
          "me_attention_fwd_x3")
    return out, lse, o3

# ... 454 lines not shown
```

Measured before the change: 8599 samples/s.

## Store 8-bit GELU-derivative in a tiled layout matching the fc2 dgrad register fragment

Adds a new ME_GG8T format that stores the quantized GELU derivative saved by the fc1 forward GEMM in 16x64 slabs, laid out to match each lane's register fragment. The fc2 dgrad epilogue then reads it with a single 128-bit buffer load per tile and skips the lane shuffles needed for the row-major 8-bit format, and the fc1 epilogue computes and packs it before the permlane swap. The block and encoder paths pick the tiled format when the resident kernel accepts it. This trims epilogue memory traffic and instruction count, but adds a new layout, padded row allocation and more kernel template variants.

Result: no change. 8675 samples/s, median of 6 (+0.9%).

```diff
diff --git a/include/metaenc.h b/include/metaenc.h
--- a/include/metaenc.h
+++ b/include/metaenc.h
@@ -14,7 +14,8 @@
        ME_F16 = 2 ,
        ME_BF16X3 = 3 ,
        ME_BF16X2 = 4 ,
-       ME_GG8 = 5  };
+       ME_GG8 = 5 ,
+       ME_GG8T = 6  };
 
 enum { ME_OK = 0, ME_ERR_ARG = -1, ME_ERR_UNSUPPORTED = -2, ME_ERR_HIP = -3, ME_ERR_WORKSPACE = -4 };
 
diff --git a/metatransformer_amd/_capi.py b/metatransformer_amd/_capi.py
--- a/metatransformer_amd/_capi.py
+++ b/metatransformer_amd/_capi.py
@@ -13,6 +13,7 @@
 ME_BF16X3 = 3
 ME_BF16X2 = 4
 ME_GG8 = 5
+ME_GG8T = 6
 ME_GEMM_NT, ME_GEMM_TN = 0, 1
 ME_ACT_NONE, ME_ACT_GELU = 0, 1
 ME_GEMM_SAVE_GELU_GRAD, ME_GEMM_AUX_IS_FACTOR = 1, 2
diff --git a/metatransformer_amd/csrc/block.hip b/metatransformer_amd/csrc/block.hip
--- a/metatransformer_amd/csrc/block.hip
+++ b/metatransformer_amd/csrc/block.hip
@@ -58,13 +58,36 @@
     return ME_OK;
 }
 
+void gemm_desc(me_gemm_desc& g, int op, int dt, int64_t M, int64_t N, int64_t K, const void* A, int64_t lda, const void* B,
+               int64_t ldb, void* C, int64_t ldc, int cdt);
+
+bool mlp_gg8_tiled(const me_block_desc* d, const Dims& s) {
+    if (d->dtype != ME_BF16) return false;
+    static char dummy_mem[64] __attribute__((aligned(64)));
+    me_gemm_desc g;
+    for (int save = 0; save < 2; ++save) {
+        gemm_desc(g, ME_GEMM_NT, ME_BF16, s.M, s.Hd, s.C, dummy_mem, s.C, dummy_mem, s.C, dummy_mem, s.Hd, ME_BF16);
+        if (save) {
+            g.bias = reinterpret_cast<const float*>(dummy_mem);
+            g.act = ME_ACT_GELU; g.flags = ME_GEMM_SAVE_GELU_GRAD; g.preact = dummy_mem; g.ldpre = s.Hd; g.preact_dtype = ME_GG8T;
+        } else {
+            g.flags = ME_GEMM_AUX_IS_FACTOR; g.aux = dummy_mem; g.ldaux = s.Hd; g.aux_dtype = ME_GG8T;
+        }
+        g.workspace = dummy_mem; g.workspace_bytes = (int64_t)1 << 40;
+        if (!me_gemm_takes_gg8(&g)) return false;
+    }
+    return true;
+}
+
 struct Saved {
     char *xn1, *qkv, *o, *x1, *xn2, *hpre, *a;
     float *mean1, *rstd1, *mean2, *rstd2, *lse;
     size_t bytes;
+    bool gg8t;
 };
 Saved carve_saved(const me_block_desc* d, const Dims& s, void* base) {
     Saved v;
+    v.gg8t = mlp_gg8_tiled(d, s);
     size_t off = 0;
     char* b = reinterpret_cast<char*>(base);
     auto take = [&](size_t n) { char* p = b + off; off += align256(n); return p; };
@@ -73,7 +96,7 @@
     v.o = take(s.M * s.C * s.esz);
     v.x1 = take(s.M * s.C * s.rsz);
     v.xn2 = take(s.M * s.C * s.esz);
-    v.hpre = take(s.M * s.Hd * s.esz);
+    v.hpre = take(v.gg8t ? (size_t)((s.M + 15) / 16 * 16) * s.Hd : s.M * s.Hd * s.esz);
     v.a = take(s.M * s.Hd * s.esz);
     v.mean1 = reinterpret_cast<float*>(take(s.M * 4));
     v.rstd1 = reinterpret_cast<float*>(take(s.M * 4));
@@ -457,7 +480,7 @@
         g.bias = d->fc1_b;
     }
     g.act = ME_ACT_GELU;
-    if (keep) { g.preact = v.hpre; g.ldpre = s.Hd; g.preact_dtype = dt; g.flags = ME_GEMM_SAVE_GELU_GRAD; }
+    if (keep) { g.preact = v.hpre; g.ldpre = s.Hd; g.preact_dtype = v.gg8t ? ME_GG8T : dt; g.flags = ME_GEMM_SAVE_GELU_GRAD; }
     g.workspace = gws; g.workspace_bytes = (int64_t)gsz;
     if ((rc = me_gemm(&g, stream))) return rc;
     gemm_desc(g, ME_GEMM_NT, dt, s.M, s.C, s.Hd, v.a, s.Hd, d->fc2_w, s.Hd, y, s.C, rdt);
@@ -529,7 +552,7 @@
 
     auto nt = [&](const void* A, int64_t K, const void* Wt, void* C, int64_t N, const void* aux) -> int {
         gemm_desc(g, ME_GEMM_NT, dt, s.M, N, K, A, K, Wt, K, C, N, dt);
-        if (aux) { g.aux = aux; g.ldaux = N; g.aux_dtype = dt; g.flags = ME_GEMM_AUX_IS_FACTOR; }
+        if (aux) { g.aux = aux; g.ldaux = N; g.aux_dtype = v.gg8t ? ME_GG8T : dt; g.flags = ME_GEMM_AUX_IS_FACTOR; }
         g.workspace = gws; g.workspace_bytes = (int64_t)gsz;
         return me_gemm(&g, stream);
     };
diff --git a/metatransformer_amd/csrc/common.h b/metatransformer_amd/csrc/common.h
--- a/metatransformer_amd/csrc/common.h
+++ b/metatransformer_amd/csrc/common.h
@@ -80,7 +80,7 @@
     ~ProfScope();
 };
 
-static inline size_t me_dtype_size(int dt) { return dt == ME_F32 ? 4 : dt == ME_GG8 ? 1 : 2; }
+static inline size_t me_dtype_size(int dt) { return dt == ME_F32 ? 4 : (dt == ME_GG8 || dt == ME_GG8T) ? 1 : 2; }
 static inline bool me_dtype_ok(int dt) { return dt == ME_F32 || dt == ME_BF16; }
 static inline bool me_storage_dtype_ok(int dt) { return me_dtype_ok(dt) || dt == ME_F16; }
 static inline bool me_out_dtype_ok(int dt) { return me_dtype_ok(dt) || dt == ME_BF16X3; }
diff --git a/metatransformer_amd/csrc/gemm.hip b/metatransformer_amd/csrc/gemm.hip
--- a/metatransformer_amd/csrc/gemm.hip
+++ b/metatransformer_amd/csrc/gemm.hip
@@ -540,9 +540,11 @@
     ME_CHECK_ARG(!(d->flags & ME_GEMM_SAVE_GELU_GRAD) || (d->act == ME_ACT_GELU && d->preact), "me_gemm: ME_GEMM_SAVE_GELU_GRAD needs act = GELU and preact");
     ME_CHECK_ARG(!(d->flags & ME_GEMM_AUX_IS_FACTOR) || d->aux, "me_gemm: ME_GEMM_AUX_IS_FACTOR needs aux");
     if (d->preact) ME_CHECK_ARG((me_dtype_ok(d->preact_dtype) && d->ldpre % 4 == 0) ||
-                                (d->preact_dtype == ME_GG8 && d->flags == ME_GEMM_SAVE_GELU_GRAD && d->ldpre % 8 == 0 && (uintptr_t)d->preact % 8 == 0), "me_gemm: bad preact");
+                                (d->preact_dtype == ME_GG8 && d->flags == ME_GEMM_SAVE_GELU_GRAD && d->ldpre % 8 == 0 && (uintptr_t)d->preact % 8 == 0) ||
+                                (d->preact_dtype == ME_GG8T && d->flags == ME_GEMM_SAVE_GELU_GRAD && d->ldpre == d->N && (uintptr_t)d->preact % 16 == 0), "me_gemm: bad preact");
     if (d->aux) ME_CHECK_ARG((me_dtype_ok(d->aux_dtype) && d->ldaux % 4 == 0) ||
-                             (d->aux_dtype == ME_GG8 && d->flags == ME_GEMM_AUX_IS_FACTOR && d->ldaux % 8 == 0 && (uintptr_t)d->aux % 8 == 0), "me_gemm: bad aux");
+                             (d->aux_dtype == ME_GG8 && d->flags == ME_GEMM_AUX_IS_FACTOR && d->ldaux % 8 == 0 && (uintptr_t)d->aux % 8 == 0) ||
+                             (d->aux_dtype == ME_GG8T && d->flags == ME_GEMM_AUX_IS_FACTOR && d->ldaux == d->N && (uintptr_t)d->aux % 16 == 0), "me_gemm: bad aux");
     if (d->residual) ME_CHECK_ARG(me_dtype_ok(d->res_dtype) && d->ldres % 4 == 0, "me_gemm: bad residual");
     p.A = d->A; p.B = d->B; p.C = d->C;
     p.M = d->M; p.N = d->N; p.K = d->K; p.lda = d->lda; p.ldb = d->ldb; p.ldc = d->ldc;
@@ -605,7 +607,7 @@
     const int cus = g3_cu_count();
     r.form = g3_form(p, cus);
     r.a_wrap = r.form.kernel == G3_ONE_TILE_WRAP;
-    r.gg8 = pl.tail_rows == 0 && r.form.kernel == G3_RESIDENT && r.form.pre == G3_PRE_GG8;
+    r.gg8 = pl.tail_rows == 0 && r.form.kernel == G3_RESIDENT && (r.form.pre == G3_PRE_GG8 || r.form.pre == G3_PRE_GG8T);
     GemmParams pu = p;
     pu.a_wrap_kt = 0;
     const G3Form fu = g3_form(pu, cus);
@@ -649,8 +651,8 @@
         ME_CHECK_ARG(r.a_wrap, "me_gemm: a_wrap_k is not available for this problem (see me_gemm_takes_a_wrap)");
     if (d->row_parts)
         ME_CHECK_ARG(r.row_parts, "me_gemm: row_parts is not available for this problem (see me_gemm_takes_row_parts)");
-    if ((d->preact && d->preact_dtype == ME_GG8) || (d->aux && d->aux_dtype == ME_GG8))
-        ME_CHECK_ARG(r.gg8, "me_gemm: ME_GG8 is not available for this problem (see me_gemm_takes_gg8)");
+    if ((d->preact && (d->preact_dtype == ME_GG8 || d->preact_dtype == ME_GG8T)) || (d->aux && (d->aux_dtype == ME_GG8 || d->aux_dtype == ME_GG8T)))
+        ME_CHECK_ARG(r.gg8, "me_gemm: ME_GG8 / ME_GG8T: the resident 256 x 256 kernel does not take this problem (see me_gemm_takes_gg8)");
 
     if (pl.family == GEMM_G3 && d->op == ME_GEMM_TN) {
         ME_CHECK_ARG(have_ws, "me_gemm(TN, g3): workspace of me_gemm_workspace_bytes() required");
diff --git a/metatransformer_amd/csrc/gemm3.hip b/metatransformer_amd/csrc/gemm3.hip
--- a/metatransformer_amd/csrc/gemm3.hip
+++ b/metatransformer_amd/csrc/gemm3.hip
@@ -170,7 +170,8 @@
                                               const __amdgpu_buffer_rsrc_t brs, int ntn, bool next_zero, unsigned* ctr, int nx,
                                               uint32_t lds_tick, int64_t next_m0 = 0, int next_rows = 0, int par = 0) {
     constexpr bool G8 = PRE == 6, G8S = G8 && EPI == 1, G8L = G8 && EPI == 6;
-    static_assert(!G8 || EPI == 1 || EPI == 6, "8-bit gelu': the fc1 forward that saves it, the fc2 dgrad that reads it");
+    constexpr bool G8T = PRE == 7, G8TS = G8T && EPI == 1, G8TL = G8T && EPI == 6;
+    static_assert(!(G8 || G8T) || EPI == 1 || EPI == 6, "8-bit gelu': the fc1 forward that saves it, the fc2 dgrad that reads it");
     constexpr bool SAVE = PRE == 1 || PRE == 2 || G8S, LNF = PRE == 3 || PRE == 5, LNP = PRE == 5, STATS = PRE == 4;
     static_assert(!STATS || EPI == 2, "row statistics: the residual epilogue");
     constexpr int NMT = HALF ? 4 : 8, WROWS = HALF ? 64 : 128;
@@ -193,7 +194,17 @@
     };
     const __amdgpu_buffer_rsrc_t crs = tile_rsrc(p.C, p.ldc);
     const __amdgpu_buffer_rsrc_t prs = SAVE ? tile_rsrc(p.preact, p.ldpre, G8S ? 1 : 2) : crs;
-    const __amdgpu_buffer_rsrc_t rrs = EPI == 2 ? tile_rsrc(p.residual, p.ldres) : (EPI == 3 || EPI == 6) ? tile_rsrc(p.aux, p.ldaux, G8L ? 1 : 2) : crs;
+    const int64_t t_nsl = p.N >> 6;
+    const int t_srows = (int)((rows + 15) >> 4), t_scols = (int)(cols >> 6);
+    auto slab_rsrc = [&](const void* base) {
+        if (!item_ok) return __builtin_amdgcn_make_buffer_rsrc(const_cast<void*>(base), 0, 0, 0x00020000);
+        return __builtin_amdgcn_make_buffer_rsrc(const_cast<char*>(reinterpret_cast<const char*>(base)) + ((m0 >> 4) * t_nsl + (n0 >> 6)) * 1024, 0,
+                                                 (int)(((t_srows - 1) * t_nsl + t_scols) * 1024), 0x00020000);
+    };
+    const __amdgpu_buffer_rsrc_t trs = G8TS ? slab_rsrc(p.preact) : G8TL ? slab_rsrc(p.aux) : crs;
+    const uint32_t toff = (G8T && wc < t_scols) ? (uint32_t)(((wr * (WROWS / 16)) * (int)t_nsl + wc) * 1024 + lane * 16) : 0x80000000u;
+    const int tstep = (int)t_nsl * 1024;
+    const __amdgpu_buffer_rsrc_t rrs = EPI == 2 ? tile_rsrc(p.residual, p.ldres) : ((EPI == 3 || EPI == 6) && !G8TL) ? tile_rsrc(p.aux, p.ldaux, G8L ? 1 : 2) : crs;
     const int rop_ld = (int)(EPI == 2 ? p.ldres : p.ldaux);
     const int colb = wc * 128 + (lane & 7) * 16;
     const bool ok = (colb >> 1) + 8 <= (int)cols;
@@ -205,6 +216,10 @@
     const int to_mem = 4 * ((lane >> 3) + 8 * ((lane >> 2) & 1) + 16 * (((lane >> 1) & 1) | ((lane & 1) << 1)));
     const int to_reg = 4 * (8 * (r & 7) + 4 * (r >> 3) + 2 * (g & 1) + (g >> 1));
     auto fetch = [&](const int mt, u32x4 (&raw)[2]) {
+        if (G8TL) {
+            raw[0] = __builtin_amdgcn_raw_buffer_load_b128(trs, (int)(toff + mt * tstep), 0, G3_POL_R);
+            return;
+        }
 #pragma unroll
         for (int h = 0; h < 2; ++h) {
             if (G8L) {
@@ -229,6 +244,16 @@
             w1 = __builtin_amdgcn_cvt_pk_u8_f32(__builtin_fmaf(b[e], 1.0f / ME_GG8_STEP, -ME_GG8_LO / ME_GG8_STEP), e, w1);
         }
         return u32x4{w0, w1, 0u, 0u};
+    };
+    auto unpack8w = [](const unsigned w) {
+        const f32x4 q = {(float)(w & 0xffu), (float)((w >> 8) & 0xffu), (float)((w >> 16) & 0xffu), (float)(w >> 24)};
+        return q * ME_GG8_STEP + ME_GG8_LO;
+    };
+    auto pack8w = [](const f32x4& a) {
+        unsigned w = 0u;
+#pragma unroll
+        for (int e = 0; e < 4; ++e) w = __builtin_amdgcn_cvt_pk_u8_f32(__builtin_fmaf(a[e], 1.0f / ME_GG8_STEP, -ME_GG8_LO / ME_GG8_STEP), e, w);
+        return w;
     };
     auto lanes2 = [](const u32x4& v, int addr) {
         u32x4 o = {0u, 0u, 0u, 0u};
@@ -297,7 +322,10 @@
     for (int mt = 0; mt < NMT; ++mt) {
         f32x4 ro[2][2];
         if (EPI == 2 || EPI == 3 || EPI == 6) {
-            if (G8L) {
+            if (G8TL) {
+                ro[0][0] = unpack8w(rowop[mt][0][0]); ro[0][1] = unpack8w(rowop[mt][0][1]);
+                ro[1][0] = unpack8w(rowop[mt][0][2]); ro[1][1] = unpack8w(rowop[mt][0][3]);
+            } else if (G8L) {
                 unpack8(lanes2(rowop[mt][0], to_reg), ro[0][0], ro[0][1]);
                 unpack8(lanes2(rowop[mt][1], to_reg), ro[1][0], ro[1][1]);
             } else {
@@ -315,6 +343,25 @@
                 v[q][0] = v[q][0] * lnf_row[mt][0] + (lnf_s.v[2 * q] * lnf_row[mt][1] + lnf_c.v[2 * q]);
                 v[q][1] = v[q][1] * lnf_row[mt][0] + (lnf_s.v[2 * q + 1] * lnf_row[mt][1] + lnf_c.v[2 * q + 1]);
             }
+        }
+        if (G8TS) {
+            u32x4 q8;
+#pragma unroll
+            for (int q = 0; q < 2; ++q) {
+#pragma unroll
+                for (int i = 0; i < 2; ++i) {
+                    f32x4 ph, ga;
+                    phi_parts4(v[q][i], ph, ga);
+                    const f32x4 dg = ph + v[q][i] * ga * 0.3989422804014327f;
+                    q8[2 * q + i] = pack8w(dg);
+                    v[q][i] *= ph;
+                }
+            }
+            __builtin_amdgcn_raw_buffer_store_b128(q8, trs, (int)(toff + mt * tstep), 0, G3_POL_P);
+        }
+        if (G8TL) { v[0][0] *= ro[0][0]; v[0][1] *= ro[0][1]; v[1][0] *= ro[1][0]; v[1][1] *= ro[1][1]; }
+#pragma unroll
+        for (int q = 0; q < 2; ++q) {
 #pragma unroll
             for (int e = 0; e < 4; ++e) {
                 const auto sw = __builtin_amdgcn_permlane16_swap(__float_as_uint(v[q][0][e]), __float_as_uint(v[q][1][e]), false, false);
@@ -322,8 +369,8 @@
                 v[q][1][e] = __uint_as_float(sw[1]);
             }
         }
-        if ((EPI == 0 || EPI == 1) && !SAVE) {
-            if (EPI == 1) {
+        if (((EPI == 0 || EPI == 1) && !SAVE) || G8T) {
+            if (EPI == 1 && !G8TS) {
                 v[0][0] = gelu_bf16_4(v[0][0]); v[0][1] = gelu_bf16_4(v[0][1]);
                 v[1][0] = gelu_bf16_4(v[1][0]); v[1][1] = gelu_bf16_4(v[1][1]);
             }
@@ -432,7 +479,7 @@
         __builtin_amdgcn_sched_barrier(0);
     }
     if (HALF) {
-        constexpr int PAD = (SAVE ? 16 : 8) + ((EPI == 2 || EPI == 6) ? 4 : EPI == 3 ? 8 : 0) ;
+        constexpr int PAD = (SAVE ? 16 : G8TS ? 12 : 8) + ((EPI == 2 || EPI == 6) ? 4 : EPI == 3 ? 8 : 0) ;
         const u32x4 z = {0u, 0u, 0u, 0u};
         const __amdgpu_buffer_rsrc_t none = __builtin_amdgcn_make_buffer_rsrc(p.C, 0, 0, 0x00020000);
 #pragma unroll
@@ -441,12 +488,12 @@
     __builtin_amdgcn_sched_barrier(0);
     g3r_set_binit(s, nb, next_zero);
     if (ctr && s.wave == 0) {
-        asm volatile("s_waitcnt vmcnt(%0)" ::"n"(2 + 4 + 16 + (SAVE ? 16 : 0) + ((EPI == 2 || EPI == 3 || EPI == 6) ? (HALF ? 8 : 16) : 0)) : "memory");
+        asm volatile("s_waitcnt vmcnt(%0)" ::"n"(2 + 4 + 16 + (SAVE ? 16 : G8TS ? 8 : 0) + ((EPI == 2 || EPI == 3 || EPI == 6) ? ((HALF || G8TL) ? 8 : 16) : 0)) : "memory");
         g3r_publish(drawn, ctr, nx, lds_tick);
     }
 }
 
-template <int EPI, int PRE> constexpr int g3r_seam() { return (PRE == 1 || PRE == 2 || (PRE == 6 && EPI == 1)) ? 32 : EPI >= 2 ? 20 : 16; }
+template <int EPI, int PRE> constexpr int g3r_seam() { return (PRE == 1 || PRE == 2 || (PRE == 6 && EPI == 1)) ? 32 : (PRE == 7 && EPI == 1) ? 24 : EPI >= 2 ? 20 : 16; }
 
 template <int EPI, int PRE, bool HI = false>
 __global__ __launch_bounds__(512) __attribute__((amdgpu_waves_per_eu(2, 2))) void gemm_g3r_kernel(const GemmParams p) {
@@ -699,12 +746,12 @@
 int launch3r_any(int epi, int pre, const GemmParams& q, int G, hipStream_t stream) {
     switch (epi) {
         case 0: return pre == G3_PRE_ROW_PARTS ? launch3r<0, G3_PRE_ROW_PARTS>(q, G, stream) : pre == G3_PRE_ROW_AFFINE ? launch3r<0, G3_PRE_ROW_AFFINE>(q, G, stream) : launch3r<0, G3_PRE_NONE>(q, G, stream);
-        case 1: return pre == G3_PRE_GG8 ? launch3r<1, G3_PRE_GG8>(q, G, stream) : pre == G3_PRE_ROW_PARTS ? launch3r<1, G3_PRE_ROW_PARTS>(q, G, stream) :
+        case 1: return pre == G3_PRE_GG8T ? launch3r<1, G3_PRE_GG8T>(q, G, stream) : pre == G3_PRE_GG8 ? launch3r<1, G3_PRE_GG8>(q, G, stream) : pre == G3_PRE_ROW_PARTS ? launch3r<1, G3_PRE_ROW_PARTS>(q, G, stream) :
                        pre == G3_PRE_ROW_AFFINE ? launch3r<1, G3_PRE_ROW_AFFINE>(q, G, stream) : pre == G3_PRE_SAVE_GELU_GRAD ? launch3r<1, G3_PRE_SAVE_GELU_GRAD>(q, G, stream) :
                        pre ? launch3r<1, G3_PRE_SAVE_PREACT>(q, G, stream) : launch3r<1, G3_PRE_NONE>(q, G, stream);
         case 2: return pre == G3_PRE_ROW_STATS ? launch3r<2, G3_PRE_ROW_STATS>(q, G, stream) : launch3r<2, G3_PRE_NONE>(q, G, stream);
         case 3: return launch3r<3, G3_PRE_NONE>(q, G, stream);
-        default: return pre == G3_PRE_GG8 ? launch3r<6, G3_PRE_GG8>(q, G, stream) : launch3r<6, G3_PRE_NONE>(q, G, stream);
+        default: return pre == G3_PRE_GG8T ? launch3r<6, G3_PRE_GG8T>(q, G, stream) : pre == G3_PRE_GG8 ? launch3r<6, G3_PRE_GG8>(q, G, stream) : launch3r<6, G3_PRE_NONE>(q, G, stream);
     }
 }
 
@@ -766,17 +813,20 @@
     }
     if (EPI == 4 && p.flags && !p.row_affine) {
         if (plain && p.flags == ME_GEMM_SAVE_GELU_GRAD && p.act == ME_ACT_GELU && p.preact && !p.aux) { f.repi = 1; f.pre = G3_PRE_SAVE_GELU_GRAD; }
-        if (plain && p.flags == ME_GEMM_AUX_IS_FACTOR && p.act == ME_ACT_NONE && p.aux && (p.aux_dtype == ME_BF16 || p.aux_dtype == ME_GG8) && !p.preact) f.repi = 6;
+        if (plain && p.flags == ME_GEMM_AUX_IS_FACTOR && p.act == ME_ACT_NONE && p.aux && (p.aux_dtype == ME_BF16 || p.aux_dtype == ME_GG8 || p.aux_dtype == ME_GG8T) && !p.preact) f.repi = 6;
     }
     if (EPI == 6) f.repi = 6;
     if (EPI == 7) { f.repi = 1; f.pre = G3_PRE_SAVE_GELU_GRAD; }
     if (f.repi == 1 && f.pre == G3_PRE_SAVE_GELU_GRAD && p.preact_dtype == ME_GG8) f.pre = G3_PRE_GG8;
     if (f.repi == 6 && p.aux_dtype == ME_GG8) f.pre = G3_PRE_GG8;
+    if (f.repi == 1 && f.pre == G3_PRE_SAVE_GELU_GRAD && p.preact_dtype == ME_GG8T) f.pre = G3_PRE_GG8T;
+    if (f.repi == 6 && p.aux_dtype == ME_GG8T) f.pre = G3_PRE_GG8T;
     if (EPI == 2 && p.row_stats) f.pre = G3_PRE_ROW_STATS;
     const int64_t ldmax = std::max(std::max(p.ldc, p.preact ? p.ldpre : 0), std::max(p.residual ? p.ldres : 0, p.aux ? p.ldaux : 0));
     const bool bf16_preact = !(f.pre == G3_PRE_SAVE_PREACT || f.pre == G3_PRE_SAVE_GELU_GRAD) || p.preact_dtype == ME_BF16;
-    const bool gg8_rows = f.pre != G3_PRE_GG8 || !p.preact || p.ldpre % 8 == 0;
-    const bool resident_only = p.row_stats || p.row_nparts || (p.preact && p.preact_dtype == ME_GG8) || (p.aux && p.aux_dtype == ME_GG8);
+    const bool gg8_rows = f.pre == G3_PRE_GG8T ? p.N % 64 == 0 : (f.pre != G3_PRE_GG8 || !p.preact || p.ldpre % 8 == 0);
+    const bool resident_only = p.row_stats || p.row_nparts || (p.preact && (p.preact_dtype == ME_GG8 || p.preact_dtype == ME_GG8T)) ||
+                               (p.aux && (p.aux_dtype == ME_GG8 || p.aux_dtype == ME_GG8T));
     if (f.repi >= 0 && !p.colscale && f.G >= 8 && f.nwg >= f.G && !split && p.alpha == 1.0f && p.c_dtype == ME_BF16 && bf16_preact && gg8_rows &&
         256 * ldmax * 2 < (1ll << 31))
         f.kernel = G3_RESIDENT;
diff --git a/metatransformer_amd/csrc/gemm_common.h b/metatransformer_amd/csrc/gemm_common.h
--- a/metatransformer_amd/csrc/gemm_common.h
+++ b/metatransformer_amd/csrc/gemm_common.h
@@ -211,7 +211,7 @@
         !p.row_affine && p.beta == 0.0f && p.out_group_rows == 0 && p.res_row_mod == 0 && p.split_k <= 1 && p.ldres % 4 == 0)
         return 8;
     if (e != 4 || me_is_planes(p.c_dtype) || p.row_affine || p.colscale || p.residual || p.beta != 0.0f || p.out_group_rows != 0 || p.res_row_mod != 0) return e;
-    if (p.flags == ME_GEMM_AUX_IS_FACTOR && p.act == ME_ACT_NONE && p.aux && (p.aux_dtype == ME_BF16 || p.aux_dtype == ME_GG8) && !p.preact) return 6;
+    if (p.flags == ME_GEMM_AUX_IS_FACTOR && p.act == ME_ACT_NONE && p.aux && (p.aux_dtype == ME_BF16 || p.aux_dtype == ME_GG8 || p.aux_dtype == ME_GG8T) && !p.preact) return 6;
     if (p.flags == ME_GEMM_SAVE_GELU_GRAD && p.act == ME_ACT_GELU && p.preact && !p.aux) return 7;
     return e;
 }
@@ -240,6 +240,7 @@
     G3_PRE_ROW_STATS = 4,
     G3_PRE_ROW_PARTS = 5,
     G3_PRE_GG8 = 6,
+    G3_PRE_GG8T = 7,
 };
 struct G3Form {
     G3Kernel kernel = G3_UNSUPPORTED;
diff --git a/metatransformer_amd/encoder.py b/metatransformer_amd/encoder.py
--- a/metatransformer_amd/encoder.py
+++ b/metatransformer_amd/encoder.py
@@ -132,9 +132,14 @@
             t1 = ops.gemm(o, cache.fwd("proj", proj_w, cdt), bias=proj_b, out_dtype=rdt, colscale=None if ls_grad else gamma1)
             x1 = ops.dropout_add(t1, x2, N, p_drop, p_path, seed + SEED_BRANCH1, colscale=gamma1 if ls_grad else None)
         xn2, mean2, rstd2 = ops.layernorm_fwd(x1, ln2_g, ln2_b, blk.eps, cdt, save_stats=need_grad)
-        hpre = torch.empty((M, fc1_w.shape[0]), dtype=cdt, device=x.device) if need_grad else None
+        hidden = fc1_w.shape[0]
+        gg8t = need_grad and stoch is None and not ls_grad and win is None and not fp8 and cdt == torch.bfloat16 and ops.gemm_takes_gg8(M, hidden, C, tiled=True)
+        hpre = None
+        if need_grad:
+            hpre = torch.empty((ops.gg8_tiled_rows(M), hidden), dtype=torch.uint8, device=x.device) if gg8t else \
+                torch.empty((M, hidden), dtype=cdt, device=x.device)
         a = ops.gemm(xn2, cache.fwd("fc1", fc1_w, cdt), bias=fc1_b, act=ME_ACT_GELU, preact=hpre,
-                     flags=ME_GEMM_SAVE_GELU_GRAD if need_grad else 0)
+                     flags=ME_GEMM_SAVE_GELU_GRAD if need_grad else 0, gg8_tiled=gg8t)
         if stoch is None and not ls_grad:
             y = ops.gemm(a, cache.fwd("fc2", fc2_w, cdt), bias=fc2_b, residual=x1, out_dtype=rdt, colscale=gamma2)
         else:
@@ -271,7 +276,8 @@
             return ops.dropout_add(dm, None, N, 0.0, 0.0, 0, out_dtype=cdt, colscale=g), dg
 
         dy_c, d_g2 = branch_grad(dy2, t2, g2, seed + SEED_BRANCH2)
-        dh = ops.gemm(dy_c, cache.transposed("fc2", fc2w, cdt), aux=hpre, flags=ME_GEMM_AUX_IS_FACTOR)
+        dh = ops.gemm(dy_c, cache.transposed("fc2", fc2w, cdt), aux=hpre, flags=ME_GEMM_AUX_IS_FACTOR,
+                      gg8_tiled=hpre.dtype == torch.uint8)
         if stoch is not None and p_drop > 0:
             dh = ops.dropout_add(dh, None, N, p_drop, 0.0, seed + SEED_MLP_HIDDEN)
         d_fc2w, d_fc2b = wgrad(dy_c, a, blk.mlp.fc2, need("fc2_w"), need("fc2_b") and ctx.has_bias[3])
diff --git a/metatransformer_amd/ops.py b/metatransformer_amd/ops.py
--- a/metatransformer_amd/ops.py
+++ b/metatransformer_amd/ops.py
@@ -89,7 +89,7 @@
          beta: float = 0.0, out_rows: Optional[int] = None, out_group: Tuple[int, int, int] = (0, 0, 0),
          want_colsum_a: bool = False, colsum_out: Optional[torch.Tensor] = None, flags: int = 0,
          row_affine: Optional[torch.Tensor] = None, col_shift: Optional[torch.Tensor] = None, want_row_stats: bool = False,
-         row_parts: Optional[torch.Tensor] = None, row_eps: float = 0.0):
+         row_parts: Optional[torch.Tensor] = None, row_eps: float = 0.0, gg8_tiled: bool = False):
     lib = _capi.load()
     _req(a, "a"); _req(b, "b")
     if a.dtype != b.dtype:
@@ -135,10 +135,10 @@
         d.colscale = ptr(colscale)
     if preact is not None:
         _req(preact, "preact")
-        d.preact, d.ldpre, d.preact_dtype = ptr(preact), preact.stride(-2), _capi.ME_GG8 if preact.dtype == torch.uint8 else dtype_code(preact.dtype)
+        d.preact, d.ldpre, d.preact_dtype = ptr(preact), preact.stride(-2), _gg8_code(gg8_tiled) if preact.dtype == torch.uint8 else dtype_code(preact.dtype)
     if aux is not None:
         _req(aux, "aux")
-        d.aux, d.ldaux, d.aux_dtype = ptr(aux), aux.stride(-2), _capi.ME_GG8 if aux.dtype == torch.uint8 else dtype_code(aux.dtype)
+        d.aux, d.ldaux, d.aux_dtype = ptr(aux), aux.stride(-2), _gg8_code(gg8_tiled) if aux.dtype == torch.uint8 else dtype_code(aux.dtype)
     if residual is not None:
         _req(residual, "residual")
         d.residual, d.ldres, d.res_dtype = ptr(residual), residual.stride(-2), dtype_code(residual.dtype)
@@ -174,7 +174,22 @@
 GG8_LO, GG8_STEP = -0.13, 1.26 / 255.0
 
 
-def gemm_takes_gg8(M: int, N: int, K: int) -> bool:
+def _gg8_code(tiled: bool) -> int:
+    return _capi.ME_GG8T if tiled else _capi.ME_GG8
+
+
+def gg8_tiled_rows(M: int) -> int:
+    return (M + 15) // 16 * 16
+
+
+def gg8_untile(buf: torch.Tensor, M: int, N: int) -> torch.Tensor:
+    sr, sc = gg8_tiled_rows(M) // 16, N // 64
+    t = buf.reshape(-1)[: sr * sc * 1024].reshape(sr, sc, 4, 16, 4, 4)
+    return t.permute(0, 3, 1, 4, 2, 5).reshape(sr * 16, N)[:M]
+
+
+def gemm_takes_gg8(M: int, N: int, K: int, tiled: bool = False) -> bool:
+    code = _gg8_code(tiled)
     lib = _capi.load()
     dev = torch.device("cuda", torch.cuda.current_device())
     dummy = torch.empty(64, dtype=torch.uint8, device=dev)
@@ -185,9 +200,9 @@
         d.A = d.B = d.C = ptr(dummy)
         d.alpha = 1.0
         if save:
-            d.act, d.flags, d.preact, d.ldpre, d.preact_dtype = _capi.ME_ACT_GELU, _capi.ME_GEMM_SAVE_GELU_GRAD, ptr(dummy), N, _capi.ME_GG8
+            d.act, d.flags, d.preact, d.ldpre, d.preact_dtype = _capi.ME_ACT_GELU, _capi.ME_GEMM_SAVE_GELU_GRAD, ptr(dummy), N, code
         else:
-            d.flags, d.aux, d.ldaux, d.aux_dtype = _capi.ME_GEMM_AUX_IS_FACTOR, ptr(dummy), N, _capi.ME_GG8
+            d.flags, d.aux, d.ldaux, d.aux_dtype = _capi.ME_GEMM_AUX_IS_FACTOR, ptr(dummy), N, code
         d.workspace, d.workspace_bytes = ptr(dummy), 1 << 40
         if not lib.me_gemm_takes_gg8(ctypes.byref(d)):
             return False
```
